# Nikhil-AI-Labs/image-super-resolution-2

Measured on AMD Instinct MI355X. Metric: output MPix/s at x4 SR (256->1024), higher is better.
Workload: dtype bf16 (bf16 MFMA operands, fp32 accumulate, fp32 activations in HBM); 1 GPU; FreqFusion x4 full 3-expert forward (HAT-L + DAT + NAFNet-SR + fusion stack), one 256x256 LR tile -> 1024x1024 per step per GPU (BASELINE configs[1]); seeded synthetic weights (172.3 M params), 1/f-noise tiles; tile=256, parallelism=tile-sharded x1, weights RCCL-broadcast once (0.0 ms), no per-tile collectives, launch=hipGraph replay, tiles_in_flight=2

## Files before the change

image-super-resolution-2_amd/build.py:

```python
from __future__ import annotations

import os
import subprocess
import sys
from concurrent.futures import ThreadPoolExecutor

HERE = os.path.dirname(os.path.abspath(__file__))
CSRC = os.path.join(HERE, "csrc")
LIB = os.path.join(HERE, "libff_hip.so")
SOURCES = ["ff_runtime.hip", "conv_gemm.hip", "conv_gemm_bf16.hip", "gemm_rows_bf16.hip", "conv3x3_halo.hip", "sgfn_tail.hip", "ocab_attn.hip", "conv3x3_small.hip", "attention.hip", "attention_bf16.hip", "win_attn_fused.hip", "chan_qkv.hip", "token_mlp.hip", "token_linear.hip", "naf_fused.hip", "naf_tail.hip", "norm_pool.hip", "dwconv.hip", "elementwise.hip",
           "resample.hip", "freq.hip", "fusion_ops.hip", "metrics.hip", "train_ops.hip", "sr_losses.hip", "augment.hip", "ff_executor.hip"]
HIPCC = os.environ.get("HIPCC", "/opt/rocm/bin/hipcc")
FLAGS = ["--offload-arch=gfx950", "-O3", "-fPIC", "-std=c++17", "-Wall", "-Wno-unused-function", "-I" + os.path.join(HERE, "build")]


def _stale() -> bool:
    if not os.path.exists(LIB):
        return True
    t = os.path.getmtime(LIB)
    deps = [os.path.join(CSRC, f) for f in os.listdir(CSRC)] + [os.path.join(HERE, "..", "include", "ff_kernels.h")]
    return any(os.path.getmtime(d) > t for d in deps)


def gen_dispatch(path: str) -> None:
    from .lib import parse_header
    protos = {n: p for n, p in parse_header().items() if p[1] and p[1][-1] == "void*" and p[0] == "int"
              and n not in ("ff_forward", "ff_create", "ff_upload")}
    names = sorted(protos)
    out = ["// generated by build.py from include/ff_kernels.h -- do not edit", f"#define FF_DISPATCH_COUNT {len(names)}",
           "static const char* const FF_DISPATCH_NAMES[FF_DISPATCH_COUNT] = {" + ", ".join(f'"{n}"' for n in names) + "};"]
    def kinds(n):
        ks = []
        for i, ty in enumerate(protos[n][1]):
            if i == len(protos[n][1]) - 1:
                ks.append("S")
            elif ty.endswith("*"):
                ks.append("P")
            elif ty in ("float", "double"):
                ks.append("F")
            else:
                ks.append("I")
        return "".join(ks)
    out.append("static const char* const FF_DISPATCH_KINDS[FF_DISPATCH_COUNT] = {" + ", ".join(f'"{kinds(n)}"' for n in names) + "};")
    for n in names:
        out.append(f'extern "C" int {n}(' + ", ".join(protos[n][1]) + ");")
    out.append("static int ff_dispatch(int id, const FFVal* v) {\n  switch (id) {")
    for k, n in enumerate(names):
        args = []
        for i, ty in enumerate(protos[n][1]):
            if ty.endswith("*"):
                args.append(f"({ty})v[{i}].p")
            elif ty in ("float", "double"):
                args.append(f"({ty})v[{i}].f")
            else:
                args.append(f"({ty})v[{i}].i")
        out.append(f"    case {k}: return {n}(" + ", ".join(args) + ");")
    out.append('    default: ff_set_error("ff_dispatch: bad entry point id %d", id); return FF_ERR_ARG;\n  }\n}')
    txt = "\n".join(out) + "\n"
    if not os.path.exists(path) or open(path).read() != txt:
        open(path, "w").write(txt)


def build(force: bool = False, verbose: bool = False) -> str:
    objdir = os.path.join(HERE, "build")
    os.makedirs(objdir, exist_ok=True)
    gen_dispatch(os.path.join(objdir, "ff_dispatch_gen.h"))
    if not force and not _stale():
        return LIB

    def cc(src):
        obj = os.path.join(objdir, src.replace(".hip", ".o"))
        cmd = [HIPCC, *FLAGS, "-c", os.path.join(CSRC, src), "-o", obj]
        r = subprocess.run(cmd, capture_output=True, text=True)
        if r.returncode != 0:
            raise RuntimeError(f"hipcc failed for {src}:\n{r.stderr}")
        if verbose and r.stderr:
            print(r.stderr, file=sys.stderr)
        return obj

    with ThreadPoolExecutor(max_workers=min(4, os.cpu_count() or 1)) as ex:
        objs = list(ex.map(cc, SOURCES))
    r = subprocess.run([HIPCC, "--offload-arch=gfx950", "-shared", "-fPIC", "-o", LIB, *objs], capture_output=True, text=True)
    if r.returncode != 0:
        raise RuntimeError(f"link failed:\n{r.stderr}")
    return LIB


if __name__ == "__main__":
    print(build(force="--force" in sys.argv, verbose=True))
```

image-super-resolution-2_amd/csrc/token_mlp.hip:

```cpp
#include "ff_common.h"

#define TM_KP 192
#define TM_NP 192
#define TM_KS 12
#define W1SLOTS 25
#define W2SLOTS 5
#define W1ROWB (W1SLOTS * 16)
#define W2ROWB (W2SLOTS * 16)
#define W1PL (32 * W1SLOTS)
#define W2PL (TM_NP * W2SLOTS)
#define W1PIECES (2 * W1PL / 64)
#define W2PIECES (2 * W2PL / 64)
#define TILE_ELEMS 6144
#define XLROWB 400

struct TokenMlpParams {
  const float* x; float* out;
  const float* gamma; const float* beta;
  const __bf16* w;
  const float* b1;
  const float* b2;
  long long M;
  int ldx, ldo, K, N, HT;
  float eps;
};

template <bool VEC4, int NTERMS>
__global__ __launch_bounds__(512) void token_mlp_kernel(TokenMlpParams p) {
  extern __shared__ __attribute__((aligned(16))) unsigned char smem[];
  constexpr int W1B = W1PL * 16, W2B = W2PL * 16;
  unsigned char* W1s = smem;
  unsigned char* W2s = smem + 2 * W1B;
  unsigned char* XLs = smem + 2 * W1B + 2 * W2B;
  float* B1s = reinterpret_cast<float*>(XLs + 8 * 32 * XLROWB);
  const int tid = threadIdx.x, lane = tid & 63, wid = tid >> 6;
  const int l31 = lane & 31, hh = lane >> 5;
  const long long tok = (long long)blockIdx.x * 256 + wid * 32 + l31;
  const bool tvalid = tok < p.M;

  int off1[4], off2[4];
#pragma unroll
  for (int i = 0; i < 4; ++i) {
    int s = (wid + 8 * i) * 64 + lane;
    if (s >= 2 * W1PL) s = 2 * W1PL - 1;
    int plane = s / W1PL, t = s - plane * W1PL, row = t / W1SLOTS, q = t - row * W1SLOTS;
    if (q > 23) q = 23;
    off1[i] = plane * TILE_ELEMS + row * 192 + q * 8;
    s = (wid + 8 * i) * 64 + lane;
    if (s >= 2 * W2PL) s = 2 * W2PL - 1;
    plane = s / W2PL; t = s - plane * W2PL; row = t / W2SLOTS; q = t - row * W2SLOTS;
    if (q > 3) q = 3;
    off2[i] = (2 + plane) * TILE_ELEMS + row * 32 + q * 8;
  }
  auto dma_w1 = [&](int ht) {
    const __bf16* rec = p.w + (long long)ht * (4 * TILE_ELEMS);
#pragma unroll
    for (int i = 0; i < 4; ++i)
      if (wid + 8 * i < W1PIECES)
        __builtin_amdgcn_global_load_lds((const __attribute__((address_space(1))) void*)(rec + off1[i]),
                                         (__attribute__((address_space(3))) void*)(W1s + (wid + 8 * i) * 1024), 16, 0, 0);
  };
  auto dma_w2 = [&](int ht) {
    const __bf16* rec = p.w + (long long)ht * (4 * TILE_ELEMS);
#pragma unroll
    for (int i = 0; i < 4; ++i)
      if (wid + 8 * i < W2PIECES)
        __builtin_amdgcn_global_load_lds((const __attribute__((address_space(1))) void*)(rec + off2[i]),
                                         (__attribute__((address_space(3))) void*)(W2s + (wid + 8 * i) * 1024), 16, 0, 0);
  };
  dma_w1(0);
  dma_w2(0);
  for (int i = tid; i < p.HT * 32; i += 512) B1s[i] = p.b1[i];

  bf16x8 xh[TM_KS];
  unsigned char* xl_row = XLs + (size_t)(wid * 32 + l31) * XLROWB + 16 * hh;
  {
    float v[TM_KS][8];
    ff_wave_rows_to_frags<3>(p.x, p.ldx, (long long)blockIdx.x * 256 + wid * 32, p.M, p.K,
                          reinterpret_cast<float*>(XLs + (size_t)wid * 32 * XLROWB), lane, v);
    float mean, rstd;
    ff_frag_ln_stats<TM_KS>(v, p.K, hh, p.eps, mean, rstd);
#pragma unroll
    for (int st = 0; st < TM_KS; ++st) {
      float f[8];
      ff_frag_ln_step(v[st], p.gamma, p.beta, 16 * st + 8 * hh, p.K, mean, rstd, f);
      bf16x8 lo;
#pragma unroll
      for (int j = 0; j < 8; ++j) {
        __bf16 h, l;
        ff_bf16_split(f[j], h, l);
        xh[st][j] = h;
        lo[j] = l;
      }
      *reinterpret_cast<bf16x8*>(xl_row + 32 * st) = lo;
    }
  }

// ... 385 lines not shown
        __builtin_amdgcn_sched_barrier(0);
        hacc = __builtin_amdgcn_mfma_f32_32x32x16_bf16(ah, xl, hacc, 0, 0, 0);
        hacc = __builtin_amdgcn_mfma_f32_32x32x16_bf16(al, xh[st], hacc, 0, 0, 0);
        hacc = __builtin_amdgcn_mfma_f32_32x32x16_bf16(ah, xh[st], hacc, 0, 0, 0);
        __builtin_amdgcn_sched_barrier(0);
      }
    }
    if (ht < 3) FF_STAMP(64, 8 + 4 * ht);
    asm volatile("s_waitcnt vmcnt(0)" ::: "memory");
    __syncthreads();
    if (ht < 3) FF_STAMP(64, 9 + 4 * ht);
    if (ht + 1 < p.HT) dma_w1(ht + 1);
    bf16x8 gh[2], gl[2];
#pragma unroll
    for (int s = 0; s < 2; ++s)
#pragma unroll
      for (int j = 0; j < 8; ++j) {
        const float g = ff_gelu_fast(hacc[8 * s + j]);
        const __bf16 h = (__bf16)g;
        gh[s][j] = h;
        gl[s][j] = (__bf16)(g - (float)h);
      }
    {
      const unsigned char* ap = W2s + l31 * W2ROWB + 16 * hh;
      bf16x8 fa[2], fl[2];
#pragma unroll
      for (int u = 0; u < 2; ++u) {
        fa[u] = *reinterpret_cast<const bf16x8*>(ap + (u >> 1) * 32 * W2ROWB + 32 * (u & 1));
        fl[u] = *reinterpret_cast<const bf16x8*>(ap + (u >> 1) * 32 * W2ROWB + 32 * (u & 1) + W2B);
      }
#pragma unroll
      for (int u = 0; u < 12; ++u) {
        const int n = u >> 1, s2 = u & 1;
        const bf16x8 ah = fa[u & 1], al = fl[u & 1];
        if (u + 2 < 12) {
          fa[u & 1] = *reinterpret_cast<const bf16x8*>(ap + ((u + 2) >> 1) * 32 * W2ROWB + 32 * ((u + 2) & 1));
          fl[u & 1] = *reinterpret_cast<const bf16x8*>(ap + ((u + 2) >> 1) * 32 * W2ROWB + 32 * ((u + 2) & 1) + W2B);
        }
        __builtin_amdgcn_sched_barrier(0);
        oacc[n] = __builtin_amdgcn_mfma_f32_32x32x16_bf16(ah, gl[s2], oacc[n], 0, 0, 0);
        oacc[n] = __builtin_amdgcn_mfma_f32_32x32x16_bf16(al, gh[s2], oacc[n], 0, 0, 0);
        oacc[n] = __builtin_amdgcn_mfma_f32_32x32x16_bf16(ah, gh[s2], oacc[n], 0, 0, 0);
        __builtin_amdgcn_sched_barrier(0);
      }
    }
    if (ht < 3) FF_STAMP(64, 10 + 4 * ht);
    asm volatile("s_waitcnt vmcnt(0)" ::: "memory");
    __syncthreads();
    if (ht < 3) FF_STAMP(64, 11 + 4 * ht);
    if (ht + 1 < p.HT) dma_w2(ht + 1);
  }
  FF_STAMP(64, 40);

  {
    float* tr = reinterpret_cast<float*>(smem) + wid * (32 * 36);
    const int tq = lane >> 3, q4 = 4 * (lane & 7);
#pragma unroll
    for (int n = 0; n < 6; ++n) {
      const int c4 = n * 32 + q4;
      const bool cok = c4 < p.N;
      const f32x4 b4 = *reinterpret_cast<const f32x4*>(p.b2 + (cok ? c4 : 0));
#pragma unroll
      for (int g = 0; g < 4; ++g) {
        f32x4 v4;
#pragma unroll
        for (int e = 0; e < 4; ++e) v4[e] = oacc[n][4 * g + e];
        *reinterpret_cast<f32x4*>(tr + l31 * 36 + 8 * g + 4 * hh) = v4;
      }
      f32x4 ov[4];
#pragma unroll
      for (int i = 0; i < 4; ++i) ov[i] = *reinterpret_cast<const f32x4*>(tr + (tq + 8 * i) * 36 + q4) + b4;
      if (cok) {
        float* op = p.out + (tok0 + tq) * p.ldo + c4;
#pragma unroll
        for (int i = 0; i < 4; ++i)
          if (tok0 + tq + 8 * i < p.M) *reinterpret_cast<f32x4*>(op + (long long)(8 * i) * p.ldo) = ov[i];
      }
    }
  }
  FF_STAMP(64, 41);
  FF_STAMP_DRAINED(64, 42);
}

#define PM_W1SLOT (13 * 1024)
#define PM_W2SLOT (15 * 1024)
#define PM_OFF_W2 (2 * PM_W1SLOT)
#define PM_PROJB (6 * PM_W1SLOT)
#define PM_PATCHB (32 * FF_XS_ROW * 4)
#define PM_OFF_PATCH PM_PROJB
#define PM_OFF_VEC (PM_OFF_PATCH + 8 * PM_PATCHB)

__global__ __launch_bounds__(512) void token_projmlp_bf16_kernel(TokenProjMlpParams p) {
  extern __shared__ __attribute__((aligned(16))) unsigned char smem[];
  float* Gs = reinterpret_cast<float*>(smem + PM_OFF_VEC);
  float* Bts = Gs + TM_KP;
  float* B1s = Bts + TM_KP;
  const int tid = threadIdx.x, lane = tid & 63, wid = tid >> 6;
  const int l31 = lane & 31, hh = lane >> 5;
  const long long tok0 = ((long long)blockIdx.y * p.wpi + blockIdx.x) * 256 + wid * 32;
  float* patch = reinterpret_cast<float*>(smem + PM_OFF_PATCH + wid * PM_PATCHB);
  FF_STAMP(64, 0);

#pragma unroll
  for (int i = 0; i < 10; ++i) {
    const int pc = wid + 8 * i;
    if (pc < 78) {
      const int tile = pc / 13, pw = pc - 13 * tile;
      int s = pw * 64 + lane;
      if (s > W1PL - 1) s = W1PL - 1;
      const int row = s / W1SLOTS;
      int q = s - row * W1SLOTS;
      if (q > 23) q = 23;
      __builtin_amdgcn_global_load_lds((const __attribute__((address_space(1))) void*)(p.wp + (long long)tile * (2 * TILE_ELEMS) + row * 192 + q * 8),
                                       (__attribute__((address_space(3))) void*)(smem + pc * 1024), 16, 0, 0);
    }
  }
  int off1[2], off2[2];
#pragma unroll
  for (int i = 0; i < 2; ++i) {
    int s = (wid + 8 * i) * 64 + lane;
    if (s > W1PL - 1) s = W1PL - 1;
    int row = s / W1SLOTS, q = s - row * W1SLOTS;
    if (q > 23) q = 23;
    off1[i] = row * 192 + q * 8;
    s = (wid + 8 * i) * 64 + lane;
    if (s > W2PL - 1) s = W2PL - 1;
    row = s / W2SLOTS; q = s - row * W2SLOTS;
    if (q > 3) q = 3;
    off2[i] = 2 * TILE_ELEMS + row * 32 + q * 8;
  }
  auto dma_mlp = [&](int ht, int slot) {
    const __bf16* rec = p.w + (long long)ht * (4 * TILE_ELEMS);
#pragma unroll
    for (int i = 0; i < 2; ++i) {
      if (wid + 8 * i < 13)
        __builtin_amdgcn_global_load_lds((const __attribute__((address_space(1))) void*)(rec + off1[i]),
                                         (__attribute__((address_space(3))) void*)(smem + slot * PM_W1SLOT + (wid + 8 * i) * 1024), 16, 0, 0);
      if (wid + 8 * i < 15)
        __builtin_amdgcn_global_load_lds((const __attribute__((address_space(1))) void*)(rec + off2[i]),
                                         (__attribute__((address_space(3))) void*)(smem + PM_OFF_W2 + slot * PM_W2SLOT + (wid + 8 * i) * 1024), 16, 0, 0);
    }
  };
  for (int i = tid; i < p.HT * 32; i += 512) B1s[i] = p.b1[i];
  if (tid < TM_KP) { Gs[tid] = tid < p.K ? p.gamma[tid] : 0.f; Bts[tid] = tid < p.K ? p.beta[tid] : 0.f; }

  bf16x8 xh[TM_KS];
  if (p.io_bf16 & 1) {
    const long long tk = tok0 + l31 < p.M ? tok0 + l31 : 0;
    const __bf16* arow = reinterpret_cast<const __bf16*>(p.att) + tk * p.lda + 8 * hh;
#pragma unroll
    for (int st = 0; st < TM_KS; ++st) {
      xh[st] = *reinterpret_cast<const bf16x8*>(arow + 16 * st);
      if (16 * st + 8 * hh + 7 >= p.K) {
#pragma unroll
        for (int j = 0; j < 8; ++j)
          if (16 * st + 8 * hh + j >= p.K) xh[st][j] = (__bf16)0.f;
      }
    }
  } else {
    float v[TM_KS][8];
    ff_wave_rows_to_frags<3>(p.att, p.lda, tok0, p.M, p.K, patch, lane, v);
#pragma unroll
    for (int st = 0; st < TM_KS; ++st)
#pragma unroll
      for (int j = 0; j < 8; ++j) xh[st][j] = (__bf16)v[st][j];
  }
  FF_STAMP(64, 1);

  const int tq = lane >> 3, q4 = 4 * (lane & 7);
  f32x4 rx[4], rc[4];
  int xo[4], co[4];
#pragma unroll
  for (int i = 0; i < 4; ++i) {
// ... 23 lines not shown
#pragma unroll
    for (int r = 0; r < 16; ++r) oacc[n][r] = bpn[(r & 3) + 8 * (r >> 2)];
    const unsigned char* ap = smem + n * PM_W1SLOT + l31 * W1ROWB + 16 * hh;
    bf16x8 fa[2];
#pragma unroll
    for (int u = 0; u < 2; ++u) fa[u] = *reinterpret_cast<const bf16x8*>(ap + 32 * u);
#pragma unroll
    for (int st = 0; st < TM_KS; ++st) {
      const bf16x8 ah = fa[st & 1];
      if (st + 2 < TM_KS) fa[st & 1] = *reinterpret_cast<const bf16x8*>(ap + 32 * (st + 2));
      __builtin_amdgcn_sched_barrier(0);
      oacc[n] = __builtin_amdgcn_mfma_f32_32x32x16_bf16(ah, xh[st], oacc[n], 0, 0, 0);
      __builtin_amdgcn_sched_barrier(0);
    }
  }
  FF_STAMP(64, 2);
  asm volatile("s_waitcnt lgkmcnt(0)" ::: "memory");
  __builtin_amdgcn_s_barrier();
  FF_STAMP(64, 3);
  dma_mlp(0, 0);
  if (p.HT > 1) dma_mlp(1, 1);
#pragma unroll
  for (int n = 0; n < 6; ++n) {
    {
      load_res(n);
      const int c4 = n * 32 + q4;
      f32x4 sc = {0.f, 0.f, 0.f, 0.f};
      if (p.c2 && c4 < p.N) sc = *reinterpret_cast<const f32x4*>(p.rs2 + (long long)blockIdx.y * p.rs2_ld + c4);
#pragma unroll
      for (int i = 0; i < 4; ++i) {
        f32x4 r0 = rx[i];
        if (p.c2) r0 += rc[i] * sc;
        *reinterpret_cast<f32x4*>(patch + (tq + 8 * i) * 36 + q4) = r0;
      }
#pragma unroll
      for (int g = 0; g < 4; ++g) {
        const f32x4 u = *reinterpret_cast<const f32x4*>(patch + l31 * 36 + 8 * g + 4 * hh);
#pragma unroll
        for (int e = 0; e < 4; ++e) oacc[n][4 * g + e] += u[e];
      }
    }
  }
  FF_STAMP(64, 4);

  {
    float s = 0.f;
#pragma unroll
    for (int n = 0; n < 6; ++n)
#pragma unroll
      for (int r = 0; r < 16; ++r) s += (n * 32 + (r & 3) + 8 * (r >> 2) + 4 * hh < p.K) ? oacc[n][r] : 0.f;
    s += __shfl_xor(s, 32);
    const float mean = s / (float)p.K;
    float qv = 0.f;
#pragma unroll
    for (int n = 0; n < 6; ++n)
#pragma unroll
      for (int r = 0; r < 16; ++r) {
        const float d = (n * 32 + (r & 3) + 8 * (r >> 2) + 4 * hh < p.K) ? oacc[n][r] - mean : 0.f;
        qv += d * d;
      }
    qv += __shfl_xor(qv, 32);
    const float rstd = 1.0f / sqrtf(qv / (float)p.K + p.eps);
#pragma unroll
    for (int n = 0; n < 6; ++n)
#pragma unroll
      for (int s2 = 0; s2 < 2; ++s2) {
#pragma unroll
        for (int g2 = 0; g2 < 2; ++g2) {
          const int c0 = n * 32 + 8 * (2 * s2 + g2) + 4 * hh;
          const f32x4 g4 = *reinterpret_cast<const f32x4*>(Gs + c0);
          const f32x4 b4 = *reinterpret_cast<const f32x4*>(Bts + c0);
#pragma unroll
          for (int e = 0; e < 4; ++e)
            xh[2 * n + s2][4 * g2 + e] = (__bf16)((oacc[n][8 * s2 + 4 * g2 + e] - mean) * rstd * g4[e] + b4[e]);
        }
        asm volatile("" : "+v"(xh[2 * n + s2]) :: "memory");
      }
  }
  FF_STAMP(64, 5);
  asm volatile("s_waitcnt vmcnt(0) lgkmcnt(0)" ::: "memory");
  __builtin_amdgcn_s_barrier();
  FF_STAMP(64, 6);

  for (int ht = 0; ht < p.HT; ++ht) {
    const int slot = ht & 1;
    f32x16 hacc;
#pragma unroll
    for (int r = 0; r < 16; ++r) hacc[r] = B1s[ht * 32 + (r & 3) + 8 * (r >> 2) + 4 * hh];
    {
      const unsigned char* ap = smem + slot * PM_W1SLOT + l31 * W1ROWB + 16 * hh;
      bf16x8 fa[2];
#pragma unroll
      for (int u = 0; u < 2; ++u) fa[u] = *reinterpret_cast<const bf16x8*>(ap + 32 * u);
#pragma unroll
      for (int st = 0; st < TM_KS; ++st) {
        const bf16x8 ah = fa[st & 1];
        if (st + 2 < TM_KS) fa[st & 1] = *reinterpret_cast<const bf16x8*>(ap + 32 * (st + 2));
        __builtin_amdgcn_sched_barrier(0);
        hacc = __builtin_amdgcn_mfma_f32_32x32x16_bf16(ah, xh[st], hacc, 0, 0, 0);
        __builtin_amdgcn_sched_barrier(0);
      }
    }
    if (ht < 3) FF_STAMP(64, 8 + 4 * ht);
    bf16x8 gh[2];
#pragma unroll
    for (int s = 0; s < 2; ++s)
#pragma unroll
      for (int j = 0; j < 8; j += 2) {
        const f32x2 g = ff_gelu_sig2((f32x2){hacc[8 * s + j], hacc[8 * s + j + 1]});
        gh[s][j] = (__bf16)g[0];
        gh[s][j + 1] = (__bf16)g[1];
      }
    if (ht < 3) FF_STAMP(64, 9 + 4 * ht);
    {
      const unsigned char* ap = smem + PM_OFF_W2 + slot * PM_W2SLOT + l31 * W2ROWB + 16 * hh;
      bf16x8 fa[2];
#pragma unroll
      for (int u = 0; u < 2; ++u) fa[u] = *reinterpret_cast<const bf16x8*>(ap + (u >> 1) * 32 * W2ROWB + 32 * (u & 1));
#pragma unroll
      for (int u = 0; u < 12; ++u) {
        const int n = u >> 1, s2 = u & 1;
        const bf16x8 ah = fa[u & 1];
        if (u + 2 < 12) fa[u & 1] = *reinterpret_cast<const bf16x8*>(ap + ((u + 2) >> 1) * 32 * W2ROWB + 32 * ((u + 2) & 1));
        __builtin_amdgcn_sched_barrier(0);
        oacc[n] = __builtin_amdgcn_mfma_f32_32x32x16_bf16(ah, gh[s2], oacc[n], 0, 0, 0);
        __builtin_amdgcn_sched_barrier(0);
      }
    }
    if (ht < 3) FF_STAMP(64, 10 + 4 * ht);
    asm volatile("s_waitcnt vmcnt(0) lgkmcnt(0)" ::: "memory");
    __builtin_amdgcn_s_barrier();
    if (ht < 3) FF_STAMP(64, 11 + 4 * ht);
    if (ht + 2 < p.HT) dma_mlp(ht + 2, slot);
  }
  FF_STAMP(64, 40);

  {
#pragma unroll
    for (int n = 0; n < 6; ++n) {
      const int c4 = n * 32 + q4;
      const bool cok = c4 < p.N;
      const f32x4 b4 = *reinterpret_cast<const f32x4*>(p.b2 + (cok ? c4 : 0));
#pragma unroll
      for (int g = 0; g < 4; ++g) {
        f32x4 v4;
#pragma unroll
        for (int e = 0; e < 4; ++e) v4[e] = oacc[n][4 * g + e];
        *reinterpret_cast<f32x4*>(patch + l31 * 36 + 8 * g + 4 * hh) = v4;
      }
      f32x4 ov[4];
#pragma unroll
      for (int i = 0; i < 4; ++i) ov[i] = *reinterpret_cast<const f32x4*>(patch + (tq + 8 * i) * 36 + q4) + b4;
      if (cok) {
        float* op = p.out + (tok0 + tq) * p.ldo + c4;
#pragma unroll
        for (int i = 0; i < 4; ++i)
          if (tok0 + tq + 8 * i < p.M) *reinterpret_cast<f32x4*>(op + (long long)(8 * i) * p.ldo) = ov[i];
      }
    }
  }
  FF_STAMP(64, 41);
  FF_STAMP_DRAINED(64, 42);
}

static int token_projmlp_launch(const float* att, int lda, const float* x, int ldx, const float* c2, int ldc, const float* c2_scale,
                                int scale_ld, int images, float* out, int ldo, long long M, int K, int hidden_tiles, const void* proj_tiles,
                                const float* proj_bias_padded, const float* gamma, const float* beta, float eps,
                                const void* mlp_tiles, const float* b1_padded, const float* b2, int nterms, int io_bf16, void* stream) {
  FF_CHECK_ARG(nterms == 1 || nterms == 3, "ff_token_projmlp: nterms must be 1 or 3");
  FF_CHECK_ARG(io_bf16 == 0 || (nterms == 1 && io_bf16 > 0 && io_bf16 < 4), "ff_token_projmlp: bf16 att / c2 rows exist for nterms == 1 only");
  FF_CHECK_ARG(!(io_bf16 & 1) || (lda % 8 == 0 && lda >= ((K + 15) / 16) * 16), "ff_token_projmlp: bf16 att rows must be 16-byte aligned and padded to a multiple of 16 channels");
  FF_CHECK_ARG(att && x && out && proj_tiles && proj_bias_padded && gamma && beta && mlp_tiles && b1_padded && b2, "ff_token_projmlp: null pointer");
  FF_CHECK_ARG(M > 0 && K > 0 && K <= TM_KP && K % 4 == 0 && hidden_tiles > 0, "ff_token_projmlp: needs K <= 192 (K %% 4 == 0)");
  FF_CHECK_ARG(lda >= K && lda % 4 == 0 && ldx >= K && ldx % 4 == 0 && ldo >= K && ldo % 4 == 0, "ff_token_projmlp: rows must be 16-byte aligned");
  FF_CHECK_ARG((((uintptr_t)att) & 15) == 0 && (((uintptr_t)x) & 15) == 0 && (((uintptr_t)out) & 15) == 0, "ff_token_projmlp: 16-byte aligned tensors");
  FF_CHECK_ARG((c2 == nullptr) == (c2_scale == nullptr), "ff_token_projmlp: c2 / c2_scale come together");
  FF_CHECK_ARG(!c2 || (ldc >= K && ldc % 4 == 0 && (((uintptr_t)c2) & 15) == 0 && (((uintptr_t)c2_scale) & 15) == 0), "ff_token_projmlp: c2 rows must be 16-byte aligned");
  FF_CHECK_ARG((((uintptr_t)proj_tiles) & 15) == 0 && (((uintptr_t)mlp_tiles) & 15) == 0 && (((uintptr_t)gamma) & 15) == 0 &&
               (((uintptr_t)beta) & 15) == 0 && (((uintptr_t)b2) & 15) == 0, "ff_token_projmlp: weights / gamma / beta / b2 must be 16-byte aligned");
  TokenProjMlpParams p;
  p.att = att; p.x = x; p.c2 = c2; p.rs2 = c2_scale; p.out = out; p.gamma = gamma; p.beta = beta;
  p.wp = (const __bf16*)proj_tiles; p.bp = proj_bias_padded; p.w = (const __bf16*)mlp_tiles; p.b1 = b1_padded; p.b2 = b2;
  p.M = M; p.lda = lda; p.ldx = ldx; p.ldc = ldc; p.ldo = ldo; p.K = K; p.N = K; p.HT = hidden_tiles; p.eps = eps; p.io_bf16 = io_bf16;
  p.wpi = (int)(((M + 255) / 256) / images); p.rs2_ld = images > 1 ? scale_ld : 0;
  FF_STAMP_ARM(p);
  const size_t lds = (size_t)(2 * W1PL + 2 * W2PL) * 16 + (size_t)8 * 32 * XLROWB + (size_t)hidden_tiles * 32 * 4;
  FF_CHECK_ARG(lds <= 160 * 1024, "ff_token_projmlp: hidden too large for the LDS image");
  const long long nblk = (M + 255) / 256;
  const dim3 grid((unsigned)(nblk / images), (unsigned)images);
  FF_CHECK_ARG(nblk < (1LL << 31), "ff_token_projmlp: grid too large");
  FF_CHECK_ARG(M * (long long)(ldx > ldc ? ldx : ldc) < (1LL << 31), "ff_token_projmlp: too many tokens for 32-bit row offsets");
  static bool attr_set = false;
  if (!attr_set) {
    hipError_t e = hipFuncSetAttribute(reinterpret_cast<const void*>(&token_projmlp_kernel), hipFuncAttributeMaxDynamicSharedMemorySize, 160 * 1024);
    if (e != hipSuccess) { ff_set_error("ff_token_projmlp: cannot raise dynamic LDS: %s", hipGetErrorString(e)); return FF_ERR_LAUNCH; }
    attr_set = true;
  }
  if (nterms == 1) {
    const size_t lds2 = (size_t)PM_OFF_VEC + (size_t)(2 * TM_KP + hidden_tiles * 32) * 4;
    FF_CHECK_ARG(lds2 <= 160 * 1024, "ff_token_projmlp: hidden too large for the LDS image");
    static bool attr2 = false;
    if (!attr2) {
      hipError_t e = hipFuncSetAttribute(reinterpret_cast<const void*>(&token_projmlp_bf16_kernel), hipFuncAttributeMaxDynamicSharedMemorySize, 160 * 1024);
      if (e != hipSuccess) { ff_set_error("ff_token_projmlp: cannot raise dynamic LDS: %s", hipGetErrorString(e)); return FF_ERR_LAUNCH; }
      attr2 = true;
    }
    hipLaunchKernelGGL(token_projmlp_bf16_kernel, grid, dim3(512), lds2, (hipStream_t)stream, p);
  } else hipLaunchKernelGGL(token_projmlp_kernel, grid, dim3(512), lds, (hipStream_t)stream, p);
  FF_LAUNCH_CHECK("ff_token_projmlp");
  return FF_OK;
}

extern "C" int ff_token_projmlp(const float* att, int lda, const float* x, int ldx, const float* c2, int ldc, const float* c2_scale,
                                float* out, int ldo, long long M, int K, int hidden_tiles, const void* proj_tiles,
                                const float* proj_bias_padded, const float* gamma, const float* beta, float eps,
                                const void* mlp_tiles, const float* b1_padded, const float* b2, int nterms, int io_bf16, void* stream) {
  return token_projmlp_launch(att, lda, x, ldx, c2, ldc, c2_scale, 0, 1, out, ldo, M, K, hidden_tiles, proj_tiles, proj_bias_padded, gamma, beta,
// ... 51 lines not shown
```

image-super-resolution-2_amd/csrc/win_attn_fused.hip:

```cpp
#include "ff_common.h"

struct WinFusedParams {
  const float* x; float* out;
  const float* gamma; const float* beta;
  const __bf16* w;
  const float* bias;
  const float* rel;
  float* xn; float* vout;
  int ldx, ldo, ldxn, ldv, o_off, v_off;
  int B, H, W, Hp, Wp, sh, sw, use_mask, nwx, nwy;
  int head0, nheads, d, K, zero_pad, rel_rows, rel_stride;
  int out_bf16, xn_bf16;
  float eps;
  FF_STAMP_MEMBER
};

#define WF_KS 12
#define WF_SLOTS 25
#define WF_ROWB (WF_SLOTS * 16)
#define WF_PL (32 * WF_SLOTS)
#define WF_PLB (WF_PL * 16)
#define WF_BUFB (2 * WF_PLB)
#define WF_TILE_ELEMS (32 * 192)
#define WF_KROWB 80
#define WF_KWAVE (2 * 32 * WF_KROWB)
#define WF_VROWB 528
#define WF_VPLB (32 * WF_VROWB)
#define WF_OFF_K (2 * WF_BUFB)
#define WF_OFF_V (WF_OFF_K + 8 * WF_KWAVE)
#define WF_OFF_REL (WF_OFF_V + 2 * WF_VPLB)
#define WF_REL_MAX 2560
#define WF_REL_PAD 4
#define WF_OFF_BS (WF_OFF_REL + (WF_REL_MAX + WF_REL_PAD) * 4)
#define WF_BS_MAX 576
#define WF_OFF_TOK (WF_OFF_BS + WF_BS_MAX * 4)
#define WF_OFF_REG (WF_OFF_TOK + 1024)
#define WF_OFF_SAME (WF_OFF_REG + 1024)
#define WF_LDS (WF_OFF_SAME + 9 * 8 * 4)
#define WF_XS_ROW 68

template <int WW, int NTERMS>
__global__ __launch_bounds__(512) void win_attn_fused_kernel(WinFusedParams p) {
  constexpr int WH = 256 / WW;
  constexpr int RS = WW == 8 ? 40 : (WW == 16 ? 48 : 64);
  constexpr int CMAX = (WH - 1) * RS + WW - 1;
  extern __shared__ __attribute__((aligned(16))) unsigned char smem[];
  unsigned char* KB = smem + WF_OFF_K;
  unsigned char* VB = smem + WF_OFF_V;
  float* REL = reinterpret_cast<float*>(smem + WF_OFF_REL);
  float* Bs = reinterpret_cast<float*>(smem + WF_OFF_BS);
  int* ktok = reinterpret_cast<int*>(smem + WF_OFF_TOK);
  int* kreg = reinterpret_cast<int*>(smem + WF_OFF_REG);
  unsigned* same = reinterpret_cast<unsigned*>(smem + WF_OFF_SAME);

  const int tid = threadIdx.x, lane = tid & 63, wid = tid >> 6;
  const int l31 = lane & 31, hh = lane >> 5;
  int bid = blockIdx.x;
  const int wx = bid % p.nwx; bid /= p.nwx;
  const int wy = bid % p.nwy;
  const int b = bid / p.nwy;
  FF_STAMP(64, 0);

  int off[4];
#pragma unroll
  for (int i = 0; i < 4; ++i) {
    int s = (wid + 8 * i) * 64 + lane;
    if (s >= 2 * WF_PL) s = 2 * WF_PL - 1;
    const int plane = s / WF_PL, t = s - plane * WF_PL, row = t / WF_SLOTS;
    int q = t - row * WF_SLOTS;
    if (q > 2 * WF_KS - 1) q = 2 * WF_KS - 1;
    off[i] = plane * WF_TILE_ELEMS + row * 192 + q * 8;
  }
  auto dma = [&](int tile, int buf) {
    const __bf16* rec = p.w + (long long)tile * (2 * WF_TILE_ELEMS);
#pragma unroll
    for (int i = 0; i < 4; ++i)
      if (wid + 8 * i < 25)
        __builtin_amdgcn_global_load_lds((const __attribute__((address_space(1))) void*)(rec + off[i]),
                                         (__attribute__((address_space(3))) void*)(smem + buf * WF_BUFB + (wid + 8 * i) * 1024), 16, 0, 0);
  };
  const int tile0 = 3 * p.head0, ntiles = 3 * p.nheads;
  dma(tile0, 0);

  if (tid < 256) {
    const int qy = wy * WH + tid / WW, qx = wx * WW + tid % WW;
    int oy = qy + p.sh, ox = qx + p.sw;
    if (oy >= p.Hp) oy -= p.Hp;
    if (ox >= p.Wp) ox -= p.Wp;
    ktok[tid] = (oy < p.H && ox < p.W) ? (b * p.H + oy) * p.W + ox : -1;
    int rid = 0;
    if (p.use_mask) {
      const int ry = qy < p.Hp - WH ? 0 : (qy < p.Hp - p.sh ? 1 : 2);
      const int rx = qx < p.Wp - WW ? 0 : (qx < p.Wp - p.sw ? 1 : 2);
      rid = 3 * ry + rx;
    }
    kreg[tid] = rid;
  }
  for (int i = tid; i < ntiles * 32; i += 512) Bs[i] = p.bias ? p.bias[tile0 * 32 + i] : 0.f;
  __syncthreads();

  const bool blk_mask = p.use_mask && (wy == p.nwy - 1 || wx == p.nwx - 1);
  if (blk_mask) {
    for (int i = wid; i < 72; i += 8) {
      const int region = i >> 3, t = i & 7;
      const unsigned long long bal = __ballot(l31 == lane && kreg[32 * t + l31] == region);
      if (lane == 0) same[i] = (unsigned)bal;
    }
    __syncthreads();
  }
  const int qi = wid * 32 + l31;
  const int mytok = ktok[qi];
  const bool tvalid = mytok >= 0;
  const int qreg_id = kreg[qi];
  const unsigned vmask = (unsigned)(__ballot(tvalid) & 0xffffffffu);
  const bool kill_pad = p.zero_pad != 0;
  FF_STAMP(64, 1);

  bf16x8 xh[WF_KS], xl[WF_KS];
  {
    float* xs = reinterpret_cast<float*>(smem + WF_OFF_K) + wid * (32 * WF_XS_ROW);
    const int rr = lane >> 4, cq = (lane & 15) * 4;
    float v[WF_KS][8];
// ... 355 lines not shown
```

image-super-resolution-2_amd/csrc/win_attn_fused_v2.inc:

```
#define W2_TILEB (32 * WF_ROWB)
#define W2_HEAD_SLOTS (3 * WF_PL)
#define W2_PIECES ((W2_HEAD_SLOTS + 63) / 64)
#define W2_WB (W2_PIECES * 1024)
#define W2_KROWB 80
#define W2_KWAVE (32 * W2_KROWB)
#define W2_KBUF (8 * W2_KWAVE)
#define W2_VROWB 528
#define W2_VBUF (32 * W2_VROWB)
#define W2_RELB ((WF_REL_MAX + WF_REL_PAD) * 4)
#define W2_OFF_K W2_WB
#define W2_OFF_V (W2_OFF_K + 2 * W2_KBUF)
#define W2_OFF_REL (W2_OFF_V + 2 * W2_VBUF)
#define W2_OFF_BS (W2_OFF_REL + 2 * W2_RELB)
#define W2_OFF_TOK (W2_OFF_BS + WF_BS_MAX * 4)
#define W2_OFF_REG (W2_OFF_TOK + 1024)
#define W2_OFF_SAME (W2_OFF_REG + 1024)
#define W2_LDS (W2_OFF_SAME + 9 * 8 * 4)

template <int WW, bool ONES>
__global__ __launch_bounds__(512) void win_attn_fused_v2_kernel(WinFusedParams p) {
  constexpr int WH = 256 / WW;
  constexpr int RS = WW == 8 ? 40 : (WW == 16 ? 48 : 64);
  constexpr int TPR = WW >= 32 ? 1 : 32 / WW;
  constexpr int WWM = WW >= 32 ? 32 : WW;
  extern __shared__ __attribute__((aligned(16))) unsigned char smem[];
  float* Bs = reinterpret_cast<float*>(smem + W2_OFF_BS);
  int* ktok = reinterpret_cast<int*>(smem + W2_OFF_TOK);
  int* kreg = reinterpret_cast<int*>(smem + W2_OFF_REG);
  unsigned* same = reinterpret_cast<unsigned*>(smem + W2_OFF_SAME);

  const int tid = threadIdx.x, lane = tid & 63, wid = tid >> 6;
  const int l31 = lane & 31, hh = lane >> 5;
  int bid = blockIdx.x;
  const int wx = bid % p.nwx; bid /= p.nwx;
  const int wy = bid % p.nwy;
  const int b = bid / p.nwy;
  FF_STAMP(64, 0);

  int woff[5];
#pragma unroll
  for (int i = 0; i < 5; ++i) {
    int s = (wid + 8 * i) * 64 + lane;
    if (s >= W2_HEAD_SLOTS) s = W2_HEAD_SLOTS - 1;
    const int tile = s / WF_PL, t = s - tile * WF_PL, row = t / WF_SLOTS;
    int q = t - row * WF_SLOTS;
    if (q > 2 * WF_KS - 1) q = 2 * WF_KS - 1;
    woff[i] = tile * (2 * WF_TILE_ELEMS) + row * 192 + q * 8;
  }
  const int reln = p.rel_rows * p.rel_stride;
  const int relpieces = (reln + 255) >> 8;
  auto dma_head = [&](int head, int buf) {
    const __bf16* rec = p.w + (long long)(3 * head) * (2 * WF_TILE_ELEMS);
#pragma unroll
    for (int i = 0; i < 5; ++i)
      if (wid + 8 * i < W2_PIECES)
        __builtin_amdgcn_global_load_lds((const __attribute__((address_space(1))) void*)(rec + woff[i]),
                                         (__attribute__((address_space(3))) void*)(smem + (wid + 8 * i) * 1024), 16, 0, 0);
    const float* src = p.rel + (long long)head * reln;
#pragma unroll
    for (int i = 0; i < 2; ++i)
      if (wid + 8 * i < relpieces) {
        int c = (wid + 8 * i) * 64 + lane;
        if (c > (reln >> 2) - 1) c = (reln >> 2) - 1;
        __builtin_amdgcn_global_load_lds((const __attribute__((address_space(1))) void*)(src + 4 * c),
                                         (__attribute__((address_space(3))) void*)(smem + W2_OFF_REL + buf * W2_RELB + WF_REL_PAD * 4 + (wid + 8 * i) * 1024), 16, 0, 0);
      }
  };
  dma_head(p.head0, 0);

  if (tid < 256) {
    const int qy = wy * WH + tid / WW, qx = wx * WW + tid % WW;
    int oy = qy + p.sh, ox = qx + p.sw;
    if (oy >= p.Hp) oy -= p.Hp;
    if (ox >= p.Wp) ox -= p.Wp;
    ktok[tid] = (oy < p.H && ox < p.W) ? (b * p.H + oy) * p.W + ox : -1;
    int rid = 0;
    if (p.use_mask) {
      const int ry = qy < p.Hp - WH ? 0 : (qy < p.Hp - p.sh ? 1 : 2);
      const int rx = qx < p.Wp - WW ? 0 : (qx < p.Wp - p.sw ? 1 : 2);
      rid = 3 * ry + rx;
    }
    kreg[tid] = rid;
  }
  for (int i = tid; i < 3 * p.nheads * 32; i += 512) Bs[i] = p.bias ? p.bias[3 * p.head0 * 32 + i] : 0.f;
  __syncthreads();
  if (ONES && tid < p.nheads) Bs[(3 * tid + 2) * 32 + 30] = 1.0f;

  const bool blk_mask = p.use_mask && (wy == p.nwy - 1 || wx == p.nwx - 1);
  if (!ONES && blk_mask) {
    for (int i = wid; i < 72; i += 8) {
      const int region = i >> 3, t = i & 7;
      const unsigned long long bal = __ballot(l31 == lane && kreg[32 * t + 31 - l31] == region);
      if (lane == 0) same[i] = (unsigned)bal;
    }
    __syncthreads();
  }
  const int qi = wid * 32 + 31 - l31;
  const int mytok = ktok[qi];
  const bool tvalid = mytok >= 0;
  const int qreg_id = kreg[qi];
  const unsigned vmask = (unsigned)(__ballot(tvalid) & 0xffffffffu);
  const bool kill_pad = p.zero_pad != 0;
  const float msy = (qreg_id / 3 == 2) ? -7.0625f : 7.0625f, msx = (qreg_id % 3 == 2) ? -7.0625f : 7.0625f;
  FF_STAMP(64, 1);

  bf16x8 xh[WF_KS];
  {
    float* xs = reinterpret_cast<float*>(smem + W2_OFF_K) + wid * (32 * WF_XS_ROW);
    const int rr = lane >> 4, cq = (lane & 15) * 4;
    float v[WF_KS][8];
    f32x4 t[3][8];
#pragma unroll
    for (int pass = 0; pass < 3; ++pass)
#pragma unroll
      for (int j = 0; j < 8; ++j) {
        const int r = 4 * j + rr, c = 64 * pass + cq;
        const int tk = ktok[wid * 32 + r];
        const bool ok = tk >= 0 && c < p.K;
        const f32x4 u = *reinterpret_cast<const f32x4*>(p.x + (ok ? (long long)tk * p.ldx + c : 0));
        t[pass][j] = ok ? u : (f32x4){0.f, 0.f, 0.f, 0.f};
      }
    const float* xrow = xs + (31 - l31) * WF_XS_ROW + 8 * hh;
#pragma unroll
    for (int pass = 0; pass < 3; ++pass) {
#pragma unroll
      for (int j = 0; j < 8; ++j) *reinterpret_cast<f32x4*>(xs + (4 * j + rr) * WF_XS_ROW + cq) = t[pass][j];
#pragma unroll
      for (int s4 = 0; s4 < 4; ++s4) {
        const f32x4 a = *reinterpret_cast<const f32x4*>(xrow + 16 * s4);
        const f32x4 c4 = *reinterpret_cast<const f32x4*>(xrow + 16 * s4 + 4);
#pragma unroll
        for (int e = 0; e < 4; ++e) { v[4 * pass + s4][e] = a[e]; v[4 * pass + s4][4 + e] = c4[e]; }
      }
    }
    asm volatile("s_waitcnt vmcnt(0)" ::: "memory");
    float mean = 0.f, rstd = 1.f;
    if (p.gamma) {
      float s = 0.f;
#pragma unroll
      for (int st = 0; st < WF_KS; ++st)
#pragma unroll
        for (int j = 0; j < 8; ++j) s += v[st][j];
      s += __shfl_xor(s, 32);
      mean = s / (float)p.K;
      float qv = 0.f;
#pragma unroll
      for (int st = 0; st < WF_KS; ++st)
#pragma unroll
        for (int j = 0; j < 8; ++j) {
          const float dd = (16 * st + 8 * hh + j < p.K) ? v[st][j] - mean : 0.f;
          qv += dd * dd;
        }
      qv += __shfl_xor(qv, 32);
      rstd = 1.0f / sqrtf(qv / (float)p.K + p.eps);
    }
#pragma unroll
    for (int st = 0; st < WF_KS; ++st) {
      const int k0 = 16 * st + 8 * hh;
      f32x4 g0 = {1.f, 1.f, 1.f, 1.f}, g1 = g0, b0 = {0.f, 0.f, 0.f, 0.f}, b1 = b0;
      if (p.gamma) {
        const int ka = k0 < p.K ? k0 : 0, kb = k0 + 4 < p.K ? k0 + 4 : 0;
        g0 = *reinterpret_cast<const f32x4*>(p.gamma + ka); b0 = *reinterpret_cast<const f32x4*>(p.beta + ka);
        g1 = *reinterpret_cast<const f32x4*>(p.gamma + kb); b1 = *reinterpret_cast<const f32x4*>(p.beta + kb);
      }
#pragma unroll
      for (int j = 0; j < 8; ++j) {
        const float gg = j < 4 ? g0[j & 3] : g1[j & 3], bb = j < 4 ? b0[j & 3] : b1[j & 3];
        const float f = (k0 + j < p.K) ? (p.gamma ? (v[st][j] - mean) * rstd * gg + bb : v[st][j]) : 0.f;
        xh[st][j] = (__bf16)f;
        v[st][j] = f;
      }
      if (p.xn && tvalid && p.xn_bf16) {
        if (k0 < p.K) *reinterpret_cast<bf16x8*>(reinterpret_cast<__bf16*>(p.xn) + (long long)mytok * p.ldxn + k0) = xh[st];
      } else if (p.xn && tvalid) {
        float* xr = p.xn + (long long)mytok * p.ldxn + k0;
        if (k0 < p.K) *reinterpret_cast<f32x4*>(xr) = (f32x4){v[st][0], v[st][1], v[st][2], v[st][3]};
        if (k0 + 4 < p.K) *reinterpret_cast<f32x4*>(xr + 4) = (f32x4){v[st][4], v[st][5], v[st][6], v[st][7]};
      }
    }
  }
  FF_STAMP(64, 2);

  const int rel_lane = ((qi / WW) + WH - 1) * RS + (qi % WW) + WW - 1 - (TPR - 1) * RS - (WWM - 1) + 4 * hh;
  const float LOG2E = 1.4426950408889634f;

  auto gemm_tile = [&](int j, bool swap, f32x16& acc) {
    const unsigned char* ap = smem + j * W2_TILEB + l31 * WF_ROWB + 16 * hh;
    bf16x8 fa[2];
#pragma unroll
    for (int u = 0; u < 2; ++u) fa[u] = *reinterpret_cast<const bf16x8*>(ap + 32 * u);
#pragma unroll
    for (int st = 0; st < WF_KS; ++st) {
      const bf16x8 ah = fa[st & 1];
      if (st + 2 < WF_KS) fa[st & 1] = *reinterpret_cast<const bf16x8*>(ap + 32 * (st + 2));
      __builtin_amdgcn_sched_barrier(0);
      if (!swap) acc = __builtin_amdgcn_mfma_f32_32x32x16_bf16(ah, xh[st], acc, 0, 0, 0);
      else acc = __builtin_amdgcn_mfma_f32_32x32x16_bf16(xh[st], ah, acc, 0, 0, 0);
      __builtin_amdgcn_sched_barrier(0);
    }
  };

  for (int hi = 0; hi < p.nheads; ++hi) {
    const int g = p.head0 + hi, buf = hi & 1;
    unsigned char* KB = smem + W2_OFF_K + buf * W2_KBUF;
    unsigned char* VB = smem + W2_OFF_V + buf * W2_VBUF;
    asm volatile("s_waitcnt lgkmcnt(0)" ::: "memory");
    __builtin_amdgcn_s_barrier();
    FF_STAMP(64, 3 + 8 * hi);
    bf16x8 qh[2];
    {
      f32x16 acc;
      const int nb = (3 * hi) * 32 + 4 * hh;
#pragma unroll
      for (int r = 0; r < 16; ++r) acc[r] = Bs[nb + (r & 3) + 8 * (r >> 2)];
      gemm_tile(0, false, acc);
      if (ONES && blk_mask && hh) { acc[14] = msy; acc[15] = msx; }
#pragma unroll
      for (int s = 0; s < 2; ++s)
#pragma unroll
        for (int j = 0; j < 8; ++j) qh[s][j] = (__bf16)acc[8 * s + j];
    }
    FF_STAMP(64, 4 + 8 * hi);
    {
      f32x16 acc;
      const int nb = (3 * hi + 1) * 32 + 4 * hh;
#pragma unroll
      for (int r = 0; r < 16; ++r) acc[r] = Bs[nb + (r & 3) + 8 * (r >> 2)];
      gemm_tile(1, false, acc);
      const bool zero = kill_pad && !tvalid;
      if (zero) {
#pragma unroll
        for (int r = 0; r < 16; ++r) acc[r] = 0.f;
      }
      if (ONES && blk_mask && hh) { acc[14] = msy; acc[15] = msx; }
      unsigned char* kmine = KB + wid * W2_KWAVE + l31 * W2_KROWB + 16 * hh;
#pragma unroll
      for (int s = 0; s < 2; ++s) {
        bf16x8 h8;
#pragma unroll
        for (int j = 0; j < 8; ++j) h8[j] = (__bf16)acc[8 * s + j];
        *reinterpret_cast<bf16x8*>(kmine + 32 * s) = h8;
      }
    }
    FF_STAMP(64, 5 + 8 * hi);
    {
      f32x16 acc;
      const float bv = Bs[(3 * hi + 2) * 32 + l31];
#pragma unroll
      for (int r = 0; r < 16; ++r) acc[r] = bv;
      gemm_tile(2, true, acc);
      if (kill_pad && !(ONES && l31 == 30)) {
#pragma unroll
        for (int r = 0; r < 16; ++r)
          if (!((vmask >> ((r & 3) + 8 * (r >> 2) + 4 * hh)) & 1u)) acc[r] = 0.f;
      }
      unsigned char* vp = VB + l31 * W2_VROWB + 64 * wid + 16 * hh;
#pragma unroll
      for (int s = 0; s < 2; ++s) {
        bf16x8 h8;
#pragma unroll
        for (int j = 0; j < 8; ++j) h8[j] = (__bf16)acc[8 * s + j];
        *reinterpret_cast<bf16x8*>(vp + 32 * s) = h8;
      }
      if (p.vout && l31 < p.d) {
#pragma unroll
        for (int r = 0; r < 16; ++r) {
          const int tk = ktok[wid * 32 + 31 - ((r & 3) + 8 * (r >> 2) + 4 * hh)];
          if (tk >= 0) p.vout[(long long)tk * p.ldv + p.v_off + g * p.d + l31] = acc[r];
        }
      }
    }
    FF_STAMP(64, 6 + 8 * hi);
    asm volatile("s_waitcnt lgkmcnt(0)" ::: "memory");
    __builtin_amdgcn_s_barrier();
    FF_STAMP(64, 7 + 8 * hi);
    if (hi + 1 < p.nheads) dma_head(g + 1, buf ^ 1);

    f32x16 o;
#pragma unroll
    for (int r = 0; r < 16; ++r) o[r] = 0.f;
    float m_run = -INFINITY, l_run = 0.f;
    unsigned rel_addr = (unsigned)(size_t)(__attribute__((address_space(3))) const void*)(smem + W2_OFF_REL + buf * W2_RELB + WF_REL_PAD * 4) + 4u * (unsigned)rel_lane;
    const unsigned char* kp = KB + l31 * W2_KROWB + 16 * hh;
    const unsigned char* vq = VB + l31 * W2_VROWB + 16 * hh;
    const unsigned* samep = same + 8 * qreg_id;
#pragma unroll 2
    for (int t = 0; t < 8; ++t, rel_addr -= 4u * TPR * RS, kp += W2_KWAVE, vq += 64) {
      unsigned ra = rel_addr;
      asm volatile("" : "+v"(ra));
      const ff_lds_cf relp = (ff_lds_cf)(size_t)ra;
      f32x16 st;
#pragma unroll
      for (int r = 0; r < 16; ++r) {
        const int c = (r & 3) + 8 * (r >> 2);
        st[r] = relp[(c / WW) * RS + (c % WW)];
      }
      bf16x8 vh2[2];
#pragma unroll
      for (int s = 0; s < 2; ++s) vh2[s] = *reinterpret_cast<const bf16x8*>(vq + 32 * s);
#pragma unroll
      for (int s = 0; s < 2; ++s) {
        const bf16x8 ah = *reinterpret_cast<const bf16x8*>(kp + 32 * s);
        st = __builtin_amdgcn_mfma_f32_32x32x16_bf16(ah, qh[s], st, 0, 0, 0);
      }
      if (!ONES && blk_mask) {
        const unsigned m = samep[t] >> (4 * hh);
#pragma unroll
        for (int r = 0; r < 16; ++r)
          st[r] += ((m >> ((r & 3) + 8 * (r >> 2))) & 1u) ? 0.f : -100.0f;
      }
      float mx = st[0];
#pragma unroll
      for (int r = 1; r < 16; ++r) mx = fmaxf(mx, st[r]);
      {
        float lo, hi;
        ff_halves(mx, lo, hi);
        mx = fmaxf(lo, hi);
      }
      if (__builtin_amdgcn_ballot_w64(mx > m_run) != 0) {
        const float m_new = fmaxf(m_run, mx);
        const float corr = __builtin_amdgcn_exp2f((m_run - m_new) * LOG2E);
#pragma unroll
        for (int r = 0; r < 16; ++r) o[r] *= corr;
        if (!ONES) l_run *= corr;
        m_run = m_new;
      }
      const float mneg = -m_run * LOG2E;
      float ls = 0.f;
#pragma unroll
      for (int s = 0; s < 2; ++s) {
        bf16x8 ph;
#pragma unroll
        for (int j = 0; j < 8; ++j) {
          const float e = __builtin_amdgcn_exp2f(__builtin_fmaf(st[8 * s + j], LOG2E, mneg));
          if (!ONES) ls += e;
          ph[j] = (__bf16)e;
        }
        o = __builtin_amdgcn_mfma_f32_32x32x16_bf16(vh2[s], ph, o, 0, 0, 0);
      }
      if (!ONES) l_run += ls;
    }
    float den;
    if (ONES) {
      float lo;
      ff_halves(o[14], lo, den);
    } else {
      den = l_run + __shfl_xor(l_run, 32);
    }
    const float inv = 1.0f / den;
    FF_STAMP(64, 8 + 8 * hi);
    asm volatile("s_waitcnt vmcnt(0)" ::: "memory");
    FF_STAMP(64, 9 + 8 * hi);

    if (tvalid && p.out_bf16) {
      typedef __bf16 bf16x2 __attribute__((ext_vector_type(2)));
      __bf16* orow = reinterpret_cast<__bf16*>(p.out) + (long long)mytok * p.ldo + p.o_off + g * p.d + 4 * hh;
#pragma unroll
      for (int i = 0; i < 4; ++i) {
        const int c = 8 * i + 4 * hh;
        if (c < p.d) *reinterpret_cast<bf16x2*>(orow + 8 * i) = (bf16x2){(__bf16)(o[4 * i] * inv), (__bf16)(o[4 * i + 1] * inv)};
        if (c + 2 < p.d) *reinterpret_cast<bf16x2*>(orow + 8 * i + 2) = (bf16x2){(__bf16)(o[4 * i + 2] * inv), (__bf16)(o[4 * i + 3] * inv)};
      }
    } else if (tvalid) {
      float* orow = p.out + (long long)mytok * p.ldo + p.o_off + g * p.d + 4 * hh;
#pragma unroll
      for (int i = 0; i < 4; ++i) {
        const int c = 8 * i + 4 * hh;
        if (c < p.d) *reinterpret_cast<float2*>(orow + 8 * i) = (float2){o[4 * i] * inv, o[4 * i + 1] * inv};
        if (c + 2 < p.d) *reinterpret_cast<float2*>(orow + 8 * i + 2) = (float2){o[4 * i + 2] * inv, o[4 * i + 3] * inv};
      }
    }
    FF_STAMP(64, 10 + 8 * hi);
  }
  FF_STAMP(64, 60);
  FF_STAMP_DRAINED(64, 61);
}
```

image-super-resolution-2_amd/experts.py:

```python
from __future__ import annotations

from typing import Dict, List, Optional

import torch

from . import ops
from .prep import (pack_conv, pack_dw, bn_scale_shift, fold_bn_after_conv, pack_token_linear, pack_naf_ffn, pack_naf_tail,
                   pack_win_attn, pack_win_rel, pack_token_projmlp, pack_chan_qkv, pack_token_linear_gated, pack_rel_overlap, pack_ocab_qkv)

T = torch.Tensor
SD = Dict[str, T]
RGB_MEAN = (0.4488, 0.4371, 0.4040)


def _ceil_to(n: int, m: int) -> int:
    return (n + m - 1) // m * m


class _Weights:

    def __init__(self, sd: SD, dev, prefix: str):
        self.sd, self.dev, self.p = sd, dev, prefix

    def __call__(self, name: str) -> T:
# ... 91 lines not shown
        self.pe_norm = (w("patch_embed.norm.weight"), w("patch_embed.norm.bias"))
        self.blocks: List[List[dict]] = []
        self.ocab: List[dict] = []
        self.gconv = []
        for g in range(groups):
            blks = []
            for b in range(depth):
                q = f"layers.{g}.residual_group.blocks.{b}."
                tbl = w(q + "attn.relative_position_bias_table")
                bias = tbl[rpi_sa].reshape(n, n, heads).permute(2, 1, 0).contiguous()
                blks.append(dict(rel=tbl.t().contiguous(),
                    n1=(w(q + "norm1.weight"), w(q + "norm1.bias")), qkv=lin(q + "attn.qkv"), proj=lin(q + "attn.proj"),
                    bias=bias, cab0=(w.conv(q + "conv_block.cab.0"), w(q + "conv_block.cab.0.bias")),
                    cab2=(w.conv(q + "conv_block.cab.2"), w(q + "conv_block.cab.2.bias")),
                    ca1=(w(q + "conv_block.cab.3.attention.1.weight").reshape(-1, 180).contiguous(), w(q + "conv_block.cab.3.attention.1.bias")),
                    ca2=(w(q + "conv_block.cab.3.attention.3.weight").reshape(180, -1).contiguous(), w(q + "conv_block.cab.3.attention.3.bias")),
                    n2=(w(q + "norm2.weight"), w(q + "norm2.bias")), fc1=lin(q + "mlp.fc1"), fc2=lin(q + "mlp.fc2"),
                    shift=0 if b % 2 == 0 else ws // 2))
            self.blocks.append(blks)
            q = f"layers.{g}.residual_group.overlap_attn."
            tbl = w(q + "relative_position_bias_table")
            self.ocab.append(dict(
                n1=(w(q + "norm1.weight"), w(q + "norm1.bias")), qkv=lin(q + "qkv"), proj=lin(q + "proj"),
                bias=tbl[rpi_oca].reshape(n, nk, heads).permute(2, 1, 0).contiguous(), rel=pack_rel_overlap(tbl, ws, self.ows),
                n2=(w(q + "norm2.weight"), w(q + "norm2.bias")), fc1=lin(q + "mlp.fc1"), fc2=lin(q + "mlp.fc2")))
            self.gconv.append((w.conv(f"layers.{g}.conv"), w(f"layers.{g}.conv.bias")))

    def _mlp(self, x: T, blk: dict) -> T:
        xn = ops.layernorm(x, *blk["n2"])
        h = ops.linear(xn, *blk["fc1"], act="gelu")
        return ops.linear(h, *blk["fc2"], res=x)

    def hab(self, x: T, blk: dict) -> T:
        _, H, W, C = x.shape
        d = C // self.heads
        fused = ops.fused_modes()
        b16 = ops.gemm_mode() == "bf16" and H * W >= 1024 and C % 4 == 0
        att = ops.empty_rows_bf16(tuple(x.shape), x.device) if b16 else ops.empty_like_rows(x)
        s = blk["shift"]
        if fused:
            relp = _packed(blk, "relp", lambda: pack_win_rel(blk["rel"], self.ws, self.ws))
            _, xn = ops.win_attn_fused(x, att, _wf(blk, self.heads, d), relp, gamma=blk["n1"][0], beta=blk["n1"][1], H=H, W=W,
                                       Hp=H, Wp=W, win=(self.ws, self.ws), shift=(s, s), use_mask=s > 0, want_xn="bf16" if b16 else True)
        else:
            xn = ops.layernorm(x, *blk["n1"])
            qkv = ops.linear(xn, *blk["qkv"])
            ops.window_attn(qkv, att, blk["bias"], q_off=0, k_off=C, v_off=2 * C, o_off=0, H=H, W=W, Hp=H, Wp=W, win=(self.ws, self.ws),
                            kwin=(self.ws, self.ws), shift=(s, s), use_mask=s > 0, heads=self.heads, d=d, scale=d ** -0.5)
        c1 = ops.conv2d(xn, *blk["cab0"], ksize=(3, 3), pad=(1, 1), act="gelu", out_bf16=b16, per_image=True)
        c2, c2mean = ops.conv2d(c1, *blk["cab2"], ksize=(3, 3), pad=(1, 1), want_pool="partials", out_bf16=b16)
        gate = ops.vec_mlp(c2mean, *blk["ca1"], "relu", *blk["ca2"], "sigmoid", post=self.conv_scale)
        if fused:
            return ops.token_projmlp(att, x, _pm(blk), blk["n2"][0], blk["n2"][1], c2=c2, c2_scale=gate if x.shape[0] > 1 else gate.reshape(-1))
        t = ops.mix2(x, c2, cb=gate)
        x = ops.linear(att, *blk["proj"], res=t)
        return self._mlp(x, blk)

    def ocab_block(self, x: T, blk: dict) -> T:
        _, H, W, C = x.shape
        d = C // self.heads
        fused = ops.fused_modes()
        rows16 = ops.gemm_mode() == "bf16" and (self.ws, self.ows, d) == (16, 24, 30) and H % 16 == 0 and W % 16 == 0
        if rows16:
            pk = _packed(blk, "qkv_r16", lambda: pack_ocab_qkv(*blk["qkv"], self.heads, d))
            qkv = ops.token_linear_rows16(x, pk, gamma=blk["n1"][0], beta=blk["n1"][1])
        elif fused:
            qkv = ops.token_linear(x, _tl(blk, "qkv"), gamma=blk["n1"][0], beta=blk["n1"][1])
        else:
            qkv = ops.linear(ops.layernorm(x, *blk["n1"]), *blk["qkv"])
        if rows16:
            att = ops.empty_rows_bf16(tuple(x.shape), x.device)
            hp = self.heads * 32
            ops.ocab_attn_rows16(qkv, att, blk["rel"], q_off=0, k_off=hp, v_off=2 * hp, H=H, W=W, heads=self.heads, d=d, ws=self.ws,
                                 ows=self.ows)
        else:
            att = ops.empty_like_rows(x)
            ops.window_attn(qkv, att, blk["bias"], q_off=0, k_off=C, v_off=2 * C, o_off=0, H=H, W=W, Hp=H, Wp=W, win=(self.ws, self.ws),
                            kwin=(self.ows, self.ows), shift=(0, 0), use_mask=False, heads=self.heads, d=d, scale=d ** -0.5)
        if fused:
            return ops.token_projmlp(att, x, _pm(blk), blk["n2"][0], blk["n2"][1])
        x = ops.linear(att, *blk["proj"], res=x)
        return self._mlp(x, blk)

    def group(self, x: T, g: int) -> T:
        y = x
        for blk in self.blocks[g]:
            y = self.hab(y, blk)
        y = self.ocab_block(y, self.ocab[g])
        return ops.conv2d(y, *self.gconv[g], ksize=(3, 3), pad=(1, 1), res=x, per_image=True)

    def forward(self, lr: T, taps: Optional[dict] = None, feats: Optional[dict] = None, out: Optional[T] = None) -> T:
        B, _, h, w = lr.shape
        Hp, Wp = _ceil_to(h, self.ws), _ceil_to(w, self.ws)
        if B > 1:
            if taps is not None:
                raise ops._lib.FFError("HatHIP.forward: taps are recorded for B == 1 only")
            nb = 1
            if ops.fused_modes():
                nb = max(1, min(int(self.max_batch_tokens) // (Hp * Wp), (2 ** 31 - 1) // (16 * Hp * Wp * 64)))
            if nb < B:
                if out is None:
                    out = torch.empty((B, 3, 4 * h, 4 * w), device=lr.device, dtype=torch.float32)
                fall = ops.empty_rows((B, Hp, Wp, self.after[0].shape[0]), lr.device) if feats is not None else None
                for b0 in range(0, B, nb):
                    self._forward_chunk(lr[b0:b0 + nb], None, {} if feats is not None else None, out[b0:b0 + nb],
                                        fall[b0:b0 + nb] if feats is not None else None)
                if feats is not None:
                    feats["hat"] = fall
                return out
        return self._forward_chunk(lr, taps, feats, out, None)

    def _forward_chunk(self, lr: T, taps: Optional[dict], feats: Optional[dict], out: Optional[T], feat_out: Optional[T]) -> T:
        _, _, h, w = lr.shape
        Hp, Wp = _ceil_to(h, self.ws), _ceil_to(w, self.ws)
        feat = self._enter(lr, Hp, Wp)
        x = ops.layernorm(feat, *self.pe_norm)
        for g in range(self.groups):
            if taps is not None and g == 0:
                y = x
                for b, blk in enumerate(self.blocks[0]):
                    y = self.hab(y, blk)
                    taps[f"hat.g0.b{b}"] = y
                y = self.ocab_block(y, self.ocab[0])
                taps["hat.g0.ocab"] = y
                x = ops.conv2d(y, *self.gconv[0], ksize=(3, 3), pad=(1, 1), res=x)
                taps["hat.g0.out"] = x
            else:
                x = self.group(x, g)
        return self._exit(x, feat, h, w, feats, out, feat_out)


def _dat_dpb_bias(sd: SD, p: str, hs: int, wsz: int, heads: int) -> T:
    import torch.nn.functional as F
    ys, xs = torch.meshgrid(torch.arange(1 - hs, hs), torch.arange(1 - wsz, wsz), indexing="ij")
    t = F.linear(torch.stack([ys.reshape(-1), xs.reshape(-1)], dim=1).float(), sd[p + ".pos_proj.weight"].float().cpu(),
                 sd[p + ".pos_proj.bias"].float().cpu())
    for j in ("pos1", "pos2", "pos3"):
        t = F.layer_norm(t, (t.shape[-1],), sd[f"{p}.{j}.0.weight"].float().cpu(), sd[f"{p}.{j}.0.bias"].float().cpu())
        t = F.linear(F.relu(t), sd[f"{p}.{j}.2.weight"].float().cpu(), sd[f"{p}.{j}.2.bias"].float().cpu())
    cy, cx = torch.meshgrid(torch.arange(hs), torch.arange(wsz), indexing="ij")
    cy, cx = cy.reshape(-1), cx.reshape(-1)
    idx = (cy[:, None] - cy[None, :] + hs - 1) * (2 * wsz - 1) + (cx[:, None] - cx[None, :] + wsz - 1)
    n = hs * wsz
    return t[idx.reshape(-1)].reshape(n, n, heads).permute(2, 1, 0).contiguous(), t.t().contiguous()


def dat_should_shift(g: int, b: int) -> bool:
    return (g % 2 == 0 and b > 0 and (b - 2) % 4 == 0) or (g % 2 != 0 and b % 4 == 0)


class DatHIP(_Trunk):

    max_batch_tokens = 262144
    name = "dat"

    def __init__(self, sd: SD, dev, prefix: str = "expert_ensemble.dat.", groups: int = 6, depth: int = 6, split=(8, 32),
                 heads: int = 6):
        w = _Weights(sd, dev, prefix)
        self.dev, self.groups, self.depth, self.split, self.heads = dev, groups, depth, split, heads
        self._load_trunk(w, dev)
        C = 180

        def lin(name):
            return w(name + ".weight"), w(name + ".bias")

        def folded_1x1(conv, bn, cin):
            wt = w(conv + ".weight").reshape(-1, cin)
            sc, sh = bn_scale_shift({k: v.to(dev) for k, v in sd.items() if k.startswith(prefix + bn)}, prefix + bn)
            return fold_bn_after_conv(wt, w(conv + ".bias"), sc, sh)

# ... 273 lines not shown
```

image-super-resolution-2_amd/ops.py:

```python
from __future__ import annotations

from typing import Dict, Optional, Tuple

import torch

from . import lib as _lib

ACT = {None: 0, "none": 0, "gelu": 1, "relu": 2, "lrelu": 3, "sigmoid": 4}
T = torch.Tensor

_PROF = None
_META = [0.0, 0.0]


def _note(flops: float = 0.0, nbytes: float = 0.0):
    _META[0] += flops
    _META[1] += nbytes


def _numel(*ts) -> float:
    return float(sum(t.numel() * (t.element_size() / 4.0) for t in ts if t is not None))


def _instrument(fn):
# ... 592 lines not shown
    xp, ldx, B, h_, w_, K = _nhwc(x, "win_attn_fused.x")
    out_bf16 = out.dtype == torch.bfloat16
    op, ldo, *_ = _nhwc(out, "win_attn_fused.out|bf16ok" if out_bf16 else "win_attn_fused.out")
    xn_bf16 = want_xn == "bf16"
    if (out_bf16 or xn_bf16) and _GEMM_MODE != "bf16":
        raise _lib.FFError("win_attn_fused: bf16 outputs exist for the plain-bf16 contraction mode only")
    if (h_, w_) != (H, W) or tuple(out.shape[:3]) != (B, H, W) or K != pk["K"]:
        raise _lib.FFError("win_attn_fused: x/out dims mismatch")
    nheads = pk["heads"] - head0 if nheads is None else nheads
    if tuple(rel_padded.shape[:2]) != (pk["heads"], 2 * win[0] - 1) or not rel_padded.is_contiguous():
        raise _lib.FFError("win_attn_fused: rel_padded must be [heads][2wh-1][stride]")
    if _GEMM_MODE not in ("bf16x3", "bf16"):
        raise _lib.FFError("win_attn_fused exists for the bf16 contraction modes only")
    xn, xnp, ldxn = None, None, 0
    if want_xn:
        xn = empty_rows_bf16(tuple(x.shape), x.device) if xn_bf16 else empty_like_rows(x)
        xnp, ldxn, _, _ = rows_view(xn, "win_attn_fused.xn|bf16ok" if xn_bf16 else "win_attn_fused.xn")
    vp, ldv = None, 0
    if v_out is not None:
        vp, ldv, vb, vh, vw, _ = _nhwc(v_out, "win_attn_fused.v_out")
        if (vb, vh, vw) != (B, H, W):
            raise _lib.FFError("win_attn_fused: v_out dims mismatch")
    _lib.check(_L().ff_win_attn_fused(xp, ldx, op, ldo, o_off, _ptr(gamma), _ptr(beta), float(eps), pk["w"].data_ptr(),
                                      pk["b"].data_ptr(), rel_padded.data_ptr(), rel_padded.shape[1], rel_padded.shape[2], B, H, W,
                                      Hp, Wp, win[0], win[1], shift[0], shift[1], int(use_mask), head0, nheads, pk["d"], K,
                                      int(zero_pad), xnp, ldxn, vp, ldv, v_off, 1 if _GEMM_MODE == "bf16" else 3, int(out_bf16), int(xn_bf16),
                                      _stream()))
    nwin = B * (Hp // win[0]) * (Wp // win[1])
    _note(2.0 * nwin * 256 * K * 3 * nheads * pk["d"] + 4.0 * nwin * nheads * 256 * 256 * pk["d"],
          4.0 * B * H * W * (K * (1 + (0 if not want_xn else (0.5 if xn_bf16 else 1.0))) + nheads * pk["d"] * ((0.5 if out_bf16 else 1.0) + (1 if v_out is not None else 0))))
    return (out, xn) if want_xn else out


def token_mlp(x: T, gamma: T, beta: T, pk: dict, eps: float = 1e-5) -> T:
    xp, ldx, rows, K = rows_view(x, "token_mlp.x")
    if K != pk["K"] or pk["N"] != K:
        raise _lib.FFError("token_mlp: shape mismatch")
    out = empty_like_rows(x)
    op_, ldo_, _, _ = rows_view(out, "token_mlp.out")
    _lib.check(_L().ff_token_mlp(xp, ldx, op_, ldo_, rows, K, pk["ht"], pk["N"], gamma.data_ptr(), beta.data_ptr(),
                                 float(eps), pk["w"].data_ptr(), pk["b1"].data_ptr(), pk["b2"].data_ptr(), _nterms(), _stream()))
    _note(4.0 * rows * K * pk["ht"] * 32, 8.0 * rows * K)
    return out


def token_projmlp(att: T, x: T, pk: dict, gamma: T, beta: T, *, c2: Optional[T] = None, c2_scale: Optional[T] = None,
                  eps: float = 1e-5) -> T:
    att_bf16 = att.dtype == torch.bfloat16
    c2_bf16 = c2 is not None and c2.dtype == torch.bfloat16
    if (att_bf16 or c2_bf16) and _GEMM_MODE != "bf16":
        raise _lib.FFError("token_projmlp: bf16 att / c2 rows exist for the plain-bf16 contraction mode only")
    ap, lda, rows, K = rows_view(att, "token_projmlp.att|bf16ok" if att_bf16 else "token_projmlp.att")
    xp, ldx, xr, xk = rows_view(x, "token_projmlp.x")
    if xr != rows or xk != K or K != pk["mlp"]["K"]:
        raise _lib.FFError("token_projmlp: shape mismatch")
    cp, ldc = None, 0
    if c2 is not None:
        cp, ldc, cr, ck = rows_view(c2, "token_projmlp.c2|bf16ok" if c2_bf16 else "token_projmlp.c2")
        if cr != rows or ck != K or c2_scale is None:
            raise _lib.FFError("token_projmlp: c2 shape mismatch")
    nimg = 1
    if c2 is not None and c2_scale.numel() != K:
        nimg = int(x.shape[0])
        if c2_scale.dim() != 2 or tuple(c2_scale.shape) != (nimg, K) or not c2_scale.is_contiguous() or rows % nimg:
            raise _lib.FFError(f"token_projmlp: c2_scale must be [{K}] or one row per image [{nimg},{K}], got {tuple(c2_scale.shape)}")
        if (rows // nimg) % 256:
            raise _lib.FFError(f"token_projmlp: a per-image gate needs images of a multiple of 256 rows, got {rows // nimg}")
    out = empty_like_rows(x)
    op_, ldo_, _, _ = rows_view(out, "token_projmlp.out")
    m = pk["mlp"]
    if nimg > 1:
        _lib.check(_L().ff_token_projmlp_images(ap, lda, xp, ldx, cp, ldc, _ptr(c2_scale), K, nimg, rows // nimg, op_, ldo_, rows, K, m["ht"],
                                                pk["proj"]["w"].data_ptr(), pk["proj"]["b"].data_ptr(), gamma.data_ptr(), beta.data_ptr(),
                                                float(eps), m["w"].data_ptr(), m["b1"].data_ptr(), m["b2"].data_ptr(), _nterms(),
                                                (1 if att_bf16 else 0) | (2 if c2_bf16 else 0), _stream()))
    else:
        _lib.check(_L().ff_token_projmlp(ap, lda, xp, ldx, cp, ldc, _ptr(c2_scale), op_, ldo_, rows, K, m["ht"], pk["proj"]["w"].data_ptr(),
                                         pk["proj"]["b"].data_ptr(), gamma.data_ptr(), beta.data_ptr(), float(eps), m["w"].data_ptr(),
                                         m["b1"].data_ptr(), m["b2"].data_ptr(), _nterms(), (1 if att_bf16 else 0) | (2 if c2_bf16 else 0), _stream()))
    _note(2.0 * rows * K * K + 4.0 * rows * K * m["ht"] * 32, 4.0 * rows * K * (2 + (0.5 if att_bf16 else 1.0) + (0 if c2 is None else (0.5 if c2_bf16 else 1.0))))
    return out


def token_linear(x: T, pk: dict, *, gamma: Optional[T] = None, beta: Optional[T] = None, eps: float = 1e-5, act=None,
                 res: Optional[T] = None, res2: Optional[T] = None, res2_scale: Optional[T] = None, want_xn: bool = False,
                 stats_range: Optional[Tuple[int, int]] = None, stats_eps: float = 1e-5):
    xp, ldx, rows, K = rows_view(x, "token_linear.x")
    if K != pk["K"]:
        raise _lib.FFError("token_linear: K mismatch")
    N = pk["N"]
    out = empty_rows(tuple(x.shape[:-1]) + (N,), x.device)
    op, ldo, _, _ = rows_view(out, "token_linear.out")
    rp, ldr, r2p, ldr2 = None, 0, None, 0
    if res is not None:
        rp, ldr, rr, rc = rows_view(res, "token_linear.res")
        if rr != rows or rc != N:
            raise _lib.FFError("token_linear: res shape mismatch")
    if res2 is not None:
        r2p, ldr2, rr, rc = rows_view(res2, "token_linear.res2")
        if rr != rows or rc != N or res2_scale is None or res2_scale.numel() != N:
            raise _lib.FFError("token_linear: res2 shape mismatch")
    xn, xnp, ldxn = None, None, 0
    if want_xn:
        if gamma is None:
            raise _lib.FFError("token_linear: want_xn needs LayerNorm parameters")
        xn = empty_like_rows(x)
        xnp, ldxn, _, _ = rows_view(xn, "token_linear.xn")
    stats, sp, slo, shi = None, None, 0, 0
    if stats_range is not None:
        slo, shi = stats_range
        stats = torch.empty((rows, 2), device=x.device, dtype=torch.float32)
        sp = stats.data_ptr()
    _lib.check(_L().ff_token_linear(xp, ldx, op, ldo, rows, K, pk["kpad"], N, pk["nt"], _ptr(gamma), _ptr(beta), float(eps),
                                    pk["w"].data_ptr(), _ptr(pk["b"]), ACT[act], rp, ldr, r2p, ldr2, _ptr(res2_scale), xnp, ldxn,
                                    sp, slo, shi, float(stats_eps), _nterms(), _stream()))
    _note(2.0 * rows * N * K, 4.0 * (rows * K * (2 if want_xn else 1) + rows * N * (1 + (res is not None) + (res2 is not None))))
    if stats is not None:
        return out, stats
    return (out, xn) if want_xn else out


def token_linear_rows16(x: T, pk: dict, *, gamma: Optional[T] = None, beta: Optional[T] = None, eps: float = 1e-5,
                        out: Optional[T] = None) -> T:
    if _GEMM_MODE != "bf16":
        raise _lib.FFError("token_linear_rows16 exists for the plain-bf16 contraction mode only")
    xp, ldx, rows, K = rows_view(x, "token_linear_rows16.x")
    if K != pk["K"]:
        raise _lib.FFError("token_linear_rows16: K mismatch")
    N = pk["N"]
    if out is None:
        out = empty_rows_bf16(tuple(x.shape[:-1]) + (N,), x.device)
    op, ldo, orows, oc = rows_view(out, "token_linear_rows16.out|bf16ok")
    if out.dtype != torch.bfloat16 or orows != rows or oc != N:
        raise _lib.FFError("token_linear_rows16: out must be bf16 rows [rows, N]")
    _lib.check(_L().ff_token_linear_rows16(xp, ldx, op, ldo, rows, K, pk["kpad"], N, pk["nt"], _ptr(gamma), _ptr(beta), float(eps),
                                           pk["w"].data_ptr(), _ptr(pk["b"]), pk["scale"].data_ptr(), ACT[None], None, 0, None, 0, None,
                                           None, 0, None, 0, 0, 0.0, 1, _stream()))
    _note(2.0 * rows * N * K, 4.0 * rows * K + 2.0 * rows * N)
    return out


def dwconv3_gate_pool(t: T, w_tap: T, bias: T):
    tp, ldi, B, H, W, C2 = _nhwc(t, "dwconv3_gate_pool.t")
    if B < 1 or C2 % 2 or tuple(w_tap.shape) != (9, C2):
        raise _lib.FFError("dwconv3_gate_pool: expects [B,H,W,2C] with B >= 1, [9, 2C] tap-major weights")
    C = C2 // 2
    out = torch.empty((B, H, W, C), device=t.device, dtype=torch.float32)
    pooled = torch.empty((B, C), device=t.device, dtype=torch.float32)
    if B == 1:
        nwork = int(_L().ff_dwconv3_gate_pool_workspace(C))
        work = torch.empty(nwork, device=t.device, dtype=torch.float32)
        _lib.check(_L().ff_dwconv3_gate_pool(tp, ldi, out.data_ptr(), C, H, W, C, w_tap.data_ptr(), bias.data_ptr(), pooled.data_ptr(),
                                             work.data_ptr(), nwork, _stream()))
    else:
        nwork = int(_L().ff_dwconv3_gate_pool_images_workspace(B, C))
        work = torch.empty(nwork, device=t.device, dtype=torch.float32)
        _lib.check(_L().ff_dwconv3_gate_pool_images(tp, ldi, out.data_ptr(), C, B, H, W, C, w_tap.data_ptr(), bias.data_ptr(),
                                                    pooled.data_ptr(), work.data_ptr(), nwork, _stream()))
    _note(2.0 * B * H * W * C2 * 9, 4.0 * B * H * W * (C2 + C))
    return out, pooled


def naf_front(x: T, pk: dict, ln_g: T, ln_b: T, w_tap: T, dw_bias: T, eps: float = 1e-6):
    xp, ldx, B, H, W, C = _nhwc(x, "naf_front.x")
    if B < 1 or C not in (64, 128) or pk["N"] != 2 * C or pk["K"] != C or pk["kpad"] != C or tuple(w_tap.shape) != (9, 2 * C):
        raise _lib.FFError("naf_front: expects [B,H,W,C] with B >= 1, C in (64, 128), conv1 packed as [2C, C], [9, 2C] tap-major weights")
# ... 658 lines not shown
    if p < 1 or p > h or p > w:
        raise _lib.FFError(f"crop_pairs_u8: patch {p} does not fit the {h}x{w} LR image")
    pl = [(int(t_), int(l_)) for t_, l_ in positions]
    if not pl:
        raise _lib.FFError("crop_pairs_u8: no positions given")
    for t_, l_ in pl:
        if not (0 <= t_ <= h - p and 0 <= l_ <= w - p):
            raise _lib.FFError(f"crop_pairs_u8: position ({t_}, {l_}) puts a {p}x{p} patch outside the {h}x{w} LR image")
    K = len(pl)
    pos = torch.tensor(pl, dtype=torch.int32).to(lr_u8.device)
    lr = torch.empty((K, 3, p, p), device=lr_u8.device, dtype=torch.float32)
    hr = torch.empty((K, 3, 4 * p, 4 * p), device=lr_u8.device, dtype=torch.float32)
    _lib.check(_L().ff_crop_pairs_u8(lr_u8.data_ptr(), hr_u8.data_ptr(), h, w, pos.data_ptr(), K, p, lr.data_ptr(), hr.data_ptr(), _stream()))
    _note(0.0, 17.0 * K * 3 * p * p * 5.0)
    return lr, hr


AA_TAPS = 16


def _cubic_aa(x: float) -> float:
    a = -0.5
    x = abs(x)
    if x < 1.0:
        return ((a + 2.0) * x - (a + 3.0)) * x * x + 1.0
    if x < 2.0:
        return ((a * x - 5.0 * a) * x + 8.0 * a) * x - 4.0 * a
    return 0.0


def aa_tables(n_in: int, n_out: int):
    import numpy as np
    if n_out < 1 or n_in < n_out:
        raise _lib.FFError(f"aa_tables: expected 1 <= n_out <= n_in, got {n_in} -> {n_out}")
    s = n_in / n_out
    span = np.zeros((n_out, 2), dtype=np.int32)
    wt = np.zeros((n_out, AA_TAPS), dtype=np.float32)
    for i in range(n_out):
        c = s * (i + 0.5)
        lo = max(int(c - 2.0 * s + 0.5), 0)
        hi = min(int(c + 2.0 * s + 0.5), n_in)
        if hi - lo > AA_TAPS:
            raise _lib.FFError(f"aa_tables: {n_in} -> {n_out} needs {hi - lo} taps, the kernel has {AA_TAPS}")
        raw = [np.float32(_cubic_aa((j + lo - c + 0.5) / s)) for j in range(hi - lo)]
        tot = np.float32(0.0)
        for v in raw:
            tot = np.float32(tot + v)
        span[i] = (lo, hi - lo)
        wt[i, :hi - lo] = [np.float32(v / tot) for v in raw]
    return span, wt


_AA_TABLES: Dict[tuple, Tuple[T, T]] = {}


def _aa_tables_dev(n_in: int, n_out: int, device) -> Tuple[T, T]:
    key = (n_in, n_out, str(device))
    ent = _AA_TABLES.get(key)
    if ent is None:
        if len(_AA_TABLES) >= 64:
            _AA_TABLES.clear()
        span, wt = aa_tables(n_in, n_out)
        ent = _AA_TABLES[key] = (torch.from_numpy(span).to(device), torch.from_numpy(wt).to(device))
    return ent


def resize_aa(x: T, size: Tuple[int, int]) -> T:
    _chk(x, "resize_aa.x")
    if x.dim() != 4 or x.shape[1] != 3 or not x.is_contiguous() or x.numel() == 0:
        raise _lib.FFError("resize_aa: expected a non-empty contiguous [B,3,H,W] tensor")
    B, C, Hi, Wi = x.shape
    Ho, Wo = (int(v) for v in size)
    if Ho < 1 or Wo < 1 or Hi != 4 * Ho or Wi != 4 * Wo:
        raise _lib.FFError(f"resize_aa: only the x1/4 ratio is built: {Hi}x{Wi} -> {Ho}x{Wo} is refused")
    span_w, wt_w = _aa_tables_dev(Wi, Wo, x.device)
    span_h, wt_h = _aa_tables_dev(Hi, Ho, x.device)
    out = torch.empty((B, C, Ho, Wo), device=x.device, dtype=torch.float32)
    _lib.check(_L().ff_resize_aa(x.data_ptr(), out.data_ptr(), B * C, Hi, Wi, Ho, Wo, span_w.data_ptr(), wt_w.data_ptr(),
                                 span_h.data_ptr(), wt_h.data_ptr(), _stream()))
    _note(0.0, 4.0 * B * C * (Hi * Wi + Ho * Wo))
    return out


for _n in ("conv2d", "sgfn_tail", "ocab_attn", "ocab_attn_rows16", "token_linear_rows16", "linear", "win_attn_fused", "token_projmlp", "token_linear_gated", "token_mlp", "token_linear", "pixel_mlp", "dwconv3_gate_pool", "naf_front", "naf_ffn", "naf_tail", "window_attn", "layernorm", "pool_mean", "vec_mlp", "dwconv2d", "dwconv3x3_ln", "mix2", "fma3", "affine",
           "nchw_to_nhwc", "nhwc_to_nchw", "resize", "avgpool2", "dct8_bands", "dwt_pass", "fft_bands", "chan_attn_weights", "chan_qkv_attn",
           "band_mha_core", "band_weight", "freq_guidance", "dynamic_gates", "fuse_blend", "tile_accum", "tile_normalize"):
    globals()[_n] = _instrument(globals()[_n])
```

include/ff_kernels.h:

```cpp
#ifndef FF_KERNELS_H
#define FF_KERNELS_H
#ifdef __cplusplus
extern "C" {
#endif

#define FF_ACT_NONE 0
#define FF_ACT_GELU 1
#define FF_ACT_RELU 2
#define FF_ACT_LRELU 3
#define FF_ACT_SIGMOID 4

const char* ff_last_error(void);
int ff_abi_version(void);
int ff_device_cu_count(void);

int ff_conv2d(const float* in, const float* w, const float* bias, const float* mul, const float* res, float* out,
              int B, int H, int W, int Cin, int ldi, int Ho, int Wo, int Cout, int ldo, int ldr, int KH, int KW,
              int sy, int sx, int py, int px, int act, float alpha, int shuffle, int tile_hint, void* stream);

int ff_conv2d_bf16s(const float* in, const void* w_hi, const void* w_lo, int Kp, int Cp, const float* bias, const float* mul,
                    const float* res, float* out, int B, int H, int W, int Cin, int ldi, int Ho, int Wo, int Cout,
                    int ldo, int ldr, int KH, int KW, int sy, int sx, int py, int px, int act, float alpha, int shuffle,
                    int nterms, int tile_hint, const float* kmul, void* stream);
int ff_conv2d_bf16s_tile(long long M, int Cout, int K, int vec4);
int ff_conv2d_bf16s_kmul_images(const float* in, int ldi, const void* w_hi, const void* w_lo, int Kp, int Cp, const float* kmul, int B,
                                int rows_per_image, const float* bias, const float* mul, const float* res, int ldr, float* out, int ldo,
                                long long M, int Cin, int Cout, int nterms, int tile_hint, void* stream);
int ff_split_bf16(const float* w, int N, int K, int Kp, int Cin, int Cp, void* hi, void* lo, void* stream);

int ff_conv2d_bf16s_wimages(const float* in, int ldi, const void* w_hi, const void* w_lo, int Kp, int Cp, int B, int rows_per_image,
                            const float* bias, const float* mul, const float* res, int ldr, float* out, int ldo, long long M, int Cin,
                            int Cout, int nterms, int tile_hint, void* stream);

int ff_gemm_rows_bf16(const void* a, int a_fp32, int lda, const void* w_hi, int Kp, const float* kmul, const float* bias,
                      const float* mul, const float* res, int ldr, void* out, int ldo, long long M, int N, int K, int gate,
                      int tile_hint, void* stream);
int ff_gemm_rows_bf16_tile(long long M, int N);
int ff_gemm_rows_bf16_kmul_images(const float* a, int lda, const void* w_hi, int Kp, const float* kmul, int B, int rows_per_image,
                                  const float* bias, const float* mul, const float* res, int ldr, float* out, int ldo, long long M,
                                  int N, int K, int tile_hint, void* stream);

int ff_conv3x3_small(const float* in, int ldi, const float* w_small, int ct, const float* bias, const float* res, int ldr,
                     float* out, int ldo, int B, int H, int W, int Cin, int Cout, int act, float alpha, void* stream);


int ff_window_attn(const float* qkv, int ldq, int q_off, int k_off, int v_off, float* out, int ldo, int o_off,
                   const float* biasT, int B, int H, int W, int Hp, int Wp, int wh, int ww, int kh, int kw,
                   int shift_h, int shift_w, int use_mask, int heads, int d, float scale, void* stream);

int ff_window_attn_bf16s(const float* qkv, int ldq, int q_off, int k_off, int v_off, float* out, int ldo, int o_off,
                         const float* biasT, int B, int H, int W, int Hp, int Wp, int wh, int ww, int kh, int kw,
                         int shift_h, int shift_w, int use_mask, int heads, int d, float scale, int nterms, const float* rel_table,
                         void* stream);

int ff_token_projmlp(const float* att, int lda, const float* x, int ldx, const float* c2, int ldc, const float* c2_scale,
                     float* out, int ldo, long long M, int K, int hidden_tiles, const void* proj_tiles,
                     const float* proj_bias_padded, const float* gamma, const float* beta, float eps,
                     const void* mlp_tiles, const float* b1_padded, const float* b2, int nterms, int io_bf16, void* stream);
int ff_token_projmlp_images(const float* att, int lda, const float* x, int ldx, const float* c2, int ldc, const float* c2_scale,
                            int scale_ld, int B, long long rows_per_image, float* out, int ldo, long long M, int K,
                            int hidden_tiles, const void* proj_tiles, const float* proj_bias_padded, const float* gamma,
                            const float* beta, float eps, const void* mlp_tiles, const float* b1_padded, const float* b2,
                            int nterms, int io_bf16, void* stream);

int ff_win_attn_fused(const float* x, int ldx, float* out, int ldo, int o_off, const float* gamma, const float* beta,
                      float eps, const void* w_tiles, const float* bias_padded, const float* rel_padded, int rel_rows,
                      int rel_stride, int B, int H, int W, int Hp, int Wp, int wh, int ww, int shift_h, int shift_w,
                      int use_mask, int head0, int nheads, int d, int K, int zero_pad_tokens, float* xn_out, int ldxn,
                      float* v_out, int ldv, int v_off, int nterms, int out_bf16, int xn_bf16, void* stream);

int ff_token_mlp(const float* x, int ldx, float* out, int ldo, long long M, int K, int hidden_tiles, int N,
                 const float* gamma, const float* beta, float eps, const void* w_tiles, const float* b1_padded,
                 const float* b2, int nterms, void* stream);

long long ff_conv3x3_halo_weight_bytes(int Cout, int Cin, int bn, int nterms);
long long ff_conv3x3_halo_pool_rows(int B, int H, int W, int Cout, int bn, int nterms);
int ff_pool_finish(const float* part, int rows, int ld, int C, float inv_count, float* out, void* stream);
int ff_conv3x3_halo(const float* in, int ldi, const void* w_img, int bn, const float* bias, const float* mul,
                    const float* res, int ldr, float* out, int ldo, int B, int H, int W, int Cin, int Cout,
                    int act, float alpha, int shuffle, float* pool_partials, int nterms, int io_bf16, void* stream);
long long ff_conv3x3_halo_images_pool_rows(int B, int H, int W, int Cout, int bn, int nterms);
int ff_conv3x3_halo_images(const float* in, int ldi, const void* w_img, int bn, const float* bias, const float* mul,
                           const float* res, int ldr, float* out, int ldo, int B, int H, int W, int Cin, int Cout,
                           int act, float alpha, int shuffle, float* pool_partials, int nterms, int io_bf16, void* stream);

int ff_token_linear(const float* x, int ldx, float* out, int ldo, long long M, int K, int kpad, int N, int n_tiles,
                    const float* gamma, const float* beta, float eps, const void* w_tiles, const float* bias_padded,
                    int act, const float* res, int ldr, const float* res2, int ldr2, const float* res2_scale,
                    float* xn_out, int ldxn, float* stats_out, int stat_lo,
                    int stat_hi, float stat_eps, int nterms, void* stream);

int ff_token_linear_rows16(const float* x, int ldx, void* out16, int ldo, long long M, int K, int kpad, int N, int n_tiles,
                           const float* gamma, const float* beta, float eps, const void* w_tiles, const float* bias_padded,
                           const float* col_scale, int act, const float* res, int ldr, const float* res2, int ldr2,
                           const float* res2_scale, float* xn_out, int ldxn, float* stats_out, int stat_lo,
                           int stat_hi, float stat_eps, int nterms, void* stream);

int ff_token_linear_gated(const float* x, int ldx, const float* x2, int ldx2, const float* cm, const float* gw1t, const float* gb1,
                          const float* gw2, float gb2, float* out, int ldo, long long M, int K, int N, int n_tiles,
                          const void* w_tiles, const float* bias_padded, const float* res, int ldr, int nterms, void* stream);
int ff_token_linear_gated_images(const float* x, int ldx, const float* x2, int ldx2, const float* cm, int B, long long rows_per_image,
                                 const float* gb1, const float* gw2, float gb2, float* out, int ldo, long long M, int K, int N, int n_tiles,
                                 const void* w_tiles, const float* bias_padded, const float* res, int ldr, int nterms, void* stream);

long long ff_dwconv3_gate_pool_workspace(int C);
int ff_dwconv3_gate_pool(const float* in, int ldi, float* out, int ldo, int H, int W, int C, const float* w_tapmajor,
                         const float* bias, float* pooled, float* work, long long work_floats, void* stream);
long long ff_dwconv3_gate_pool_images_workspace(int B, int C);
int ff_dwconv3_gate_pool_images(const float* in, int ldi, float* out, int ldo, int B, int H, int W, int C, const float* w_tapmajor,
                                const float* bias, float* pooled, float* work, long long work_floats, void* stream);

long long ff_naf_front_workspace(int H, int W, int C);
int ff_naf_front(const float* x, int ldx, int H, int W, int C, const float* ln_gamma, const float* ln_beta, float eps,
                 const void* w1_tiles, const float* b1, const float* dw_tapmajor, const float* dw_bias, float* out, int ldo,
                 float* pooled, float* work, long long work_floats, int nterms, void* stream);
long long ff_naf_front_images_workspace(int B, int H, int W, int C);
int ff_naf_front_images(const float* x, int ldx, int B, int H, int W, int C, const float* ln_gamma, const float* ln_beta, float eps,
                        const void* w1_tiles, const float* b1, const float* dw_tapmajor, const float* dw_bias, float* out, int ldo,
                        float* pooled, float* work, long long work_floats, int nterms, void* stream);
int ff_naf_ffn(const float* y, int ldy, float* out, int ldo, long long M, int C, const float* gamma_ln, const float* beta_ln,
               float eps, const void* w_tiles, const float* b4, const float* b5, const float* out_scale, int nterms, void* stream);

int ff_naf_tail(const float* g, int ldg, const float* x, int ldx, float* out, int ldo, long long M, int C, const float* sca,
                const float* b3, const float* beta, const float* gamma_ln, const float* beta_ln, float eps, const void* w_frags,
                const float* b4, const float* b5, const float* out_scale, void* stream);
int ff_naf_tail_images(const float* g, int ldg, const float* x, int ldx, float* out, int ldo, long long M, int C, const float* sca,
                       int B, int rows_per_image, const float* b3, const float* beta, const float* gamma_ln, const float* beta_ln,
                       float eps, const void* w_frags, const float* b4, const float* b5, const float* out_scale, void* stream);

int ff_layernorm(const float* in, int ldi, float* out, int ldo, long long rows, int C, const float* gamma,
                 const float* beta, float eps, void* stream);
int ff_layernorm_bf16out(const float* in, int ldi, void* out, int ldo, long long rows, int C, const float* gamma,
                         const float* beta, float eps, void* stream);

int ff_pool_mean(const float* in, int ld, int B, long long P, int C, float* out, float* work, long long work_floats,
                 void* stream);
long long ff_pool_mean_workspace(int B, long long P, int C);

int ff_vec_mlp(const float* in, int B, int Cin, const float* W1, const float* b1, int Ch, int act1, const float* W2,
               const float* b2, int Cout, int act2, float post, float* out, void* stream);

int ff_pool_partial_rows(long long P);
int ff_pool_partials(const float* in, int ld, long long P, int C, float* part, long long part_floats, void* stream);
long long ff_pool_partials_images_rows(int B, long long P);
int ff_pool_partials_images(const float* in, int ld, int B, long long P, int C, float* part, long long part_floats, void* stream);

int ff_pool_vec_mlp(const float* part, int rows, int ld, float inv_count, int Cin, const float* W1, const float* b1, int Ch,
                    int act1, const float* W2, const float* b2, int Cout, int act2, float post, float* out, float* pooled_out,
                    void* stream);
int ff_pool_vec_mlp_images(const float* part, int B, int rows, int ld, float inv_count, int Cin, const float* W1, const float* b1,
                           int Ch, int act1, const float* W2, const float* b2, int Cout, int act2, float post, float* out,
                           float* pooled_out, void* stream);
// ... 184 lines not shown
```

Baseline: 26.81 output MPix/s.

## Fuse HAB tail projection/MLP with next block's window attention in one kernel

Adds a hab_link kernel that runs one HAB block's output projection, residual with the gated CAB branch, LayerNorm and MLP, then continues into the next block's LayerNorm and windowed attention inside the same workgroup. Each workgroup owns one 16x16 window, so the tokens stay in LDS and registers between the two stages. The goal is to drop the HBM round trip of x and the extra launch between blocks. The costs are a very large, specialised kernel limited to six heads of dim 30, K=180 and 16x16 windows, with the shifted-window token mapping applied inside the MLP stage and heavy LDS reuse that could lower occupancy.

```diff
diff --git a/image-super-resolution-2_amd/build.py b/image-super-resolution-2_amd/build.py
--- a/image-super-resolution-2_amd/build.py
+++ b/image-super-resolution-2_amd/build.py
@@ -8,7 +8,7 @@
 HERE = os.path.dirname(os.path.abspath(__file__))
 CSRC = os.path.join(HERE, "csrc")
 LIB = os.path.join(HERE, "libff_hip.so")
-SOURCES = ["ff_runtime.hip", "conv_gemm.hip", "conv_gemm_bf16.hip", "gemm_rows_bf16.hip", "conv3x3_halo.hip", "sgfn_tail.hip", "ocab_attn.hip", "conv3x3_small.hip", "attention.hip", "attention_bf16.hip", "win_attn_fused.hip", "chan_qkv.hip", "token_mlp.hip", "token_linear.hip", "naf_fused.hip", "naf_tail.hip", "norm_pool.hip", "dwconv.hip", "elementwise.hip",
+SOURCES = ["ff_runtime.hip", "conv_gemm.hip", "conv_gemm_bf16.hip", "gemm_rows_bf16.hip", "conv3x3_halo.hip", "sgfn_tail.hip", "ocab_attn.hip", "conv3x3_small.hip", "attention.hip", "attention_bf16.hip", "win_attn_fused.hip", "hab_link.hip", "chan_qkv.hip", "token_mlp.hip", "token_linear.hip", "naf_fused.hip", "naf_tail.hip", "norm_pool.hip", "dwconv.hip", "elementwise.hip",
            "resample.hip", "freq.hip", "fusion_ops.hip", "metrics.hip", "train_ops.hip", "sr_losses.hip", "augment.hip", "ff_executor.hip"]
 HIPCC = os.environ.get("HIPCC", "/opt/rocm/bin/hipcc")
 FLAGS = ["--offload-arch=gfx950", "-O3", "-fPIC", "-std=c++17", "-Wall", "-Wno-unused-function", "-I" + os.path.join(HERE, "build")]
diff --git a/image-super-resolution-2_amd/csrc/hab_link.hip b/image-super-resolution-2_amd/csrc/hab_link.hip
--- /dev/null
+++ b/image-super-resolution-2_amd/csrc/hab_link.hip
@@ -0,0 +1,388 @@
+#include "ff_common.h"
+#include "token_mlp_layout.h"
+#include "win_attn_layout.h"
+
+#define HL_OFF_VEC PM_OFF_VEC
+#define HL_K 180
+#define HL_HEADS 6
+
+struct HabLinkParams {
+  const __bf16* a_att; const float* a_x; const __bf16* a_c2; const float* a_rs2; float* a_out;
+  const float* a_gamma; const float* a_beta; const __bf16* a_wp; const float* a_bp; const __bf16* a_w; const float* a_b1; const float* a_b2;
+  int a_lda, a_ldx, a_ldc, a_ldo, a_rs2_ld, HT;
+  float a_eps;
+  float* out; const float* gamma; const float* beta; const __bf16* w; const float* bias; const float* rel; float* xn;
+  int ldo, ldxn, o_off, H, W, sh, sw, use_mask, nwx, nwy, rel_rows, rel_stride;
+  int K;
+  float eps;
+  static constexpr int d = 30, head0 = 0, nheads = HL_HEADS, out_bf16 = 1, xn_bf16 = 1, ldv = 0, v_off = 0;
+  static constexpr float* vout = nullptr;
+  FF_STAMP_MEMBER
+};
+
+#define HL_LDS (HL_OFF_VEC + (2 * TM_KP + 12 * 32) * 4)
+static_assert(HL_LDS <= 160 * 1024, "LDS image too large");
+static_assert(W2_LDS <= PM_OFF_VEC, "the attention's tables must stay below phase A's vectors");
+static_assert(W2_WB <= PM_PROJB && W2_OFF_K + 8 * 32 * WF_XS_ROW * 4 <= W2_OFF_REL, "hand-over patches must clear the weight image and the bias tables");
+
+__global__ __launch_bounds__(512) void hab_link_kernel(HabLinkParams p) {
+  constexpr int WW = 16, WH = 16, RS = 48, TPR = 2, WWM = 16;
+  constexpr bool ONES = true;
+  extern __shared__ __attribute__((aligned(16))) unsigned char smem[];
+  float* Gs = reinterpret_cast<float*>(smem + HL_OFF_VEC);
+  float* Bts = Gs + TM_KP;
+  float* B1s = Bts + TM_KP;
+  float* Bs = reinterpret_cast<float*>(smem + W2_OFF_BS);
+  unsigned* same = reinterpret_cast<unsigned*>(smem + W2_OFF_SAME);
+  const int* ktok = nullptr;
+  const int tid = threadIdx.x, lane = tid & 63, wid = tid >> 6;
+  const int l31 = lane & 31, hh = lane >> 5;
+  int bid = blockIdx.x;
+  const int wx = bid % p.nwx; bid /= p.nwx;
+  const int wy = bid % p.nwy;
+  const int b = bid / p.nwy;
+  float* patch = reinterpret_cast<float*>(smem + PM_OFF_PATCH + wid * PM_PATCHB);
+  auto tok_of = [&](int pos) {
+    int oy = wy * WH + (pos >> 4) + p.sh, ox = wx * WW + (pos & 15) + p.sw;
+    if (oy >= p.H) oy -= p.H;
+    if (ox >= p.W) ox -= p.W;
+    return (b * p.H + oy) * p.W + ox;
+  };
+  FF_STAMP(128, 0);
+
+#pragma unroll
+  for (int i = 0; i < 10; ++i) {
+    const int pc = wid + 8 * i;
+    if (pc < 78) {
+      const int tile = pc / 13, pw = pc - 13 * tile;
+      int s = pw * 64 + lane;
+      if (s > W1PL - 1) s = W1PL - 1;
+      const int row = s / W1SLOTS;
+      int q = s - row * W1SLOTS;
+      if (q > 23) q = 23;
+      __builtin_amdgcn_global_load_lds((const __attribute__((address_space(1))) void*)(p.a_wp + (long long)tile * (2 * TILE_ELEMS) + row * 192 + q * 8),
+                                       (__attribute__((address_space(3))) void*)(smem + pc * 1024), 16, 0, 0);
+    }
+  }
+  int off1[2], off2[2];
+#pragma unroll
+  for (int i = 0; i < 2; ++i) {
+    int s = (wid + 8 * i) * 64 + lane;
+    if (s > W1PL - 1) s = W1PL - 1;
+    int row = s / W1SLOTS, q = s - row * W1SLOTS;
+    if (q > 23) q = 23;
+    off1[i] = row * 192 + q * 8;
+    s = (wid + 8 * i) * 64 + lane;
+    if (s > W2PL - 1) s = W2PL - 1;
+    row = s / W2SLOTS; q = s - row * W2SLOTS;
+    if (q > 3) q = 3;
+    off2[i] = 2 * TILE_ELEMS + row * 32 + q * 8;
+  }
+  auto dma_mlp = [&](int ht, int slot) {
+    const __bf16* rec = p.a_w + (long long)ht * (4 * TILE_ELEMS);
+#pragma unroll
+    for (int i = 0; i < 2; ++i) {
+      if (wid + 8 * i < 13)
+        __builtin_amdgcn_global_load_lds((const __attribute__((address_space(1))) void*)(rec + off1[i]),
+                                         (__attribute__((address_space(3))) void*)(smem + slot * PM_W1SLOT + (wid + 8 * i) * 1024), 16, 0, 0);
+      if (wid + 8 * i < 15)
+        __builtin_amdgcn_global_load_lds((const __attribute__((address_space(1))) void*)(rec + off2[i]),
+                                         (__attribute__((address_space(3))) void*)(smem + PM_OFF_W2 + slot * PM_W2SLOT + (wid + 8 * i) * 1024), 16, 0, 0);
+    }
+  };
+  for (int i = tid; i < p.HT * 32; i += 512) B1s[i] = p.a_b1[i];
+  if (tid < TM_KP) { Gs[tid] = tid < p.K ? p.a_gamma[tid] : 0.f; Bts[tid] = tid < p.K ? p.a_beta[tid] : 0.f; }
+
+  bf16x8 xh[TM_KS];
+  {
+    const __bf16* arow = p.a_att + tok_of(wid * 32 + l31) * p.a_lda + 8 * hh;
+#pragma unroll
+    for (int st = 0; st < TM_KS; ++st) {
+      xh[st] = *reinterpret_cast<const bf16x8*>(arow + 16 * st);
+      if (16 * st + 8 * hh + 7 >= p.K) {
+#pragma unroll
+        for (int j = 0; j < 8; ++j)
+          if (16 * st + 8 * hh + j >= p.K) xh[st][j] = (__bf16)0.f;
+      }
+    }
+  }
+  FF_STAMP(128, 1);
+
+  const int tq = lane >> 3, q4 = 4 * (lane & 7);
+  f32x4 rx[4], rc[4];
+  int xo[4], co[4];
+#pragma unroll
+  for (int i = 0; i < 4; ++i) {
+    const int t = tok_of(wid * 32 + tq + 8 * i);
+    xo[i] = t * p.a_ldx + q4;
+    co[i] = t * p.a_ldc + q4;
+  }
+  auto load_res = [&](int n) {
+    const int cn = (n * 32 + q4 < p.K) ? n * 32 : -q4;
+#pragma unroll
+    for (int i = 0; i < 4; ++i) {
+      rx[i] = *reinterpret_cast<const f32x4*>(p.a_x + (xo[i] + cn));
+      const bf16x4 h4 = *reinterpret_cast<const bf16x4*>(p.a_c2 + (co[i] + cn));
+      rc[i] = (f32x4){(float)h4[0], (float)h4[1], (float)h4[2], (float)h4[3]};
+    }
+  };
+  asm volatile("s_waitcnt vmcnt(0) lgkmcnt(0)" ::: "memory");
+  __builtin_amdgcn_s_barrier();
+
+  f32x16 oacc[6];
+#pragma unroll
+  for (int n = 0; n < 6; ++n) {
+    const float* bpn = p.a_bp + n * 32 + 4 * hh;
+#pragma unroll
+    for (int r = 0; r < 16; ++r) oacc[n][r] = bpn[(r & 3) + 8 * (r >> 2)];
+    const unsigned char* ap = smem + n * PM_W1SLOT + l31 * W1ROWB + 16 * hh;
+    bf16x8 fa[2];
+#pragma unroll
+    for (int u = 0; u < 2; ++u) fa[u] = *reinterpret_cast<const bf16x8*>(ap + 32 * u);
+#pragma unroll
+    for (int st = 0; st < TM_KS; ++st) {
+      const bf16x8 ah = fa[st & 1];
+      if (st + 2 < TM_KS) fa[st & 1] = *reinterpret_cast<const bf16x8*>(ap + 32 * (st + 2));
+      __builtin_amdgcn_sched_barrier(0);
+      oacc[n] = __builtin_amdgcn_mfma_f32_32x32x16_bf16(ah, xh[st], oacc[n], 0, 0, 0);
+      __builtin_amdgcn_sched_barrier(0);
+    }
+  }
+  FF_STAMP(128, 2);
+  asm volatile("s_waitcnt lgkmcnt(0)" ::: "memory");
+  __builtin_amdgcn_s_barrier();
+  FF_STAMP(128, 3);
+  dma_mlp(0, 0);
+  if (p.HT > 1) dma_mlp(1, 1);
+#pragma unroll
+  for (int n = 0; n < 6; ++n) {
+    load_res(n);
+    const int c4 = n * 32 + q4;
+    f32x4 sc = {0.f, 0.f, 0.f, 0.f};
+    if (c4 < p.K) sc = *reinterpret_cast<const f32x4*>(p.a_rs2 + (long long)b * p.a_rs2_ld + c4);
+#pragma unroll
+    for (int i = 0; i < 4; ++i) {
+      f32x4 r0 = rx[i];
+      r0 += rc[i] * sc;
+      *reinterpret_cast<f32x4*>(patch + (tq + 8 * i) * 36 + q4) = r0;
+    }
+#pragma unroll
+    for (int g = 0; g < 4; ++g) {
+      const f32x4 u = *reinterpret_cast<const f32x4*>(patch + l31 * 36 + 8 * g + 4 * hh);
+#pragma unroll
+      for (int e = 0; e < 4; ++e) oacc[n][4 * g + e] += u[e];
+    }
+  }
+  FF_STAMP(128, 4);
+
+  {
+    float s = 0.f;
+#pragma unroll
+    for (int n = 0; n < 6; ++n)
+#pragma unroll
+      for (int r = 0; r < 16; ++r) s += (n * 32 + (r & 3) + 8 * (r >> 2) + 4 * hh < p.K) ? oacc[n][r] : 0.f;
+    s += __shfl_xor(s, 32);
+    const float mean = s / (float)p.K;
+    float qv = 0.f;
+#pragma unroll
+    for (int n = 0; n < 6; ++n)
+#pragma unroll
+      for (int r = 0; r < 16; ++r) {
+        const float d = (n * 32 + (r & 3) + 8 * (r >> 2) + 4 * hh < p.K) ? oacc[n][r] - mean : 0.f;
+        qv += d * d;
+      }
+    qv += __shfl_xor(qv, 32);
+    const float rstd = 1.0f / sqrtf(qv / (float)p.K + p.a_eps);
+#pragma unroll
+    for (int n = 0; n < 6; ++n)
+#pragma unroll
+      for (int s2 = 0; s2 < 2; ++s2) {
+#pragma unroll
+        for (int g2 = 0; g2 < 2; ++g2) {
+          const int c0 = n * 32 + 8 * (2 * s2 + g2) + 4 * hh;
+          const f32x4 g4 = *reinterpret_cast<const f32x4*>(Gs + c0);
+          const f32x4 b4 = *reinterpret_cast<const f32x4*>(Bts + c0);
+#pragma unroll
+          for (int e = 0; e < 4; ++e)
+            xh[2 * n + s2][4 * g2 + e] = (__bf16)((oacc[n][8 * s2 + 4 * g2 + e] - mean) * rstd * g4[e] + b4[e]);
+        }
+        asm volatile("" : "+v"(xh[2 * n + s2]) :: "memory");
+      }
+  }
+  FF_STAMP(128, 5);
+  asm volatile("s_waitcnt vmcnt(0) lgkmcnt(0)" ::: "memory");
+  __builtin_amdgcn_s_barrier();
+  FF_STAMP(128, 6);
+
+#define PM_STAMP(i) FF_STAMP(128, i)
+#include "token_projmlp_bf16_mlp.inc"
+#undef PM_STAMP
+  FF_STAMP(128, 40);
+
+  int woff[5];
+#pragma unroll
+  for (int i = 0; i < 5; ++i) {
+    int s = (wid + 8 * i) * 64 + lane;
+    if (s >= W2_HEAD_SLOTS) s = W2_HEAD_SLOTS - 1;
+    const int tile = s / WF_PL, t = s - tile * WF_PL, row = t / WF_SLOTS;
+    int q = t - row * WF_SLOTS;
+    if (q > 2 * WF_KS - 1) q = 2 * WF_KS - 1;
+    woff[i] = tile * (2 * WF_TILE_ELEMS) + row * 192 + q * 8;
+  }
+  const int reln = p.rel_rows * p.rel_stride;
+  const int relpieces = (reln + 255) >> 8;
+  auto dma_head = [&](int head, int buf) {
+    const __bf16* rec = p.w + (long long)(3 * head) * (2 * WF_TILE_ELEMS);
+#pragma unroll
+    for (int i = 0; i < 5; ++i)
+      if (wid + 8 * i < W2_PIECES)
+        __builtin_amdgcn_global_load_lds((const __attribute__((address_space(1))) void*)(rec + woff[i]),
+                                         (__attribute__((address_space(3))) void*)(smem + (wid + 8 * i) * 1024), 16, 0, 0);
+    const float* src = p.rel + (long long)head * reln;
+#pragma unroll
+    for (int i = 0; i < 2; ++i)
+      if (wid + 8 * i < relpieces) {
+        int c = (wid + 8 * i) * 64 + lane;
+        if (c > (reln >> 2) - 1) c = (reln >> 2) - 1;
+        __builtin_amdgcn_global_load_lds((const __attribute__((address_space(1))) void*)(src + 4 * c),
+                                         (__attribute__((address_space(3))) void*)(smem + W2_OFF_REL + buf * W2_RELB + WF_REL_PAD * 4 + (wid + 8 * i) * 1024), 16, 0, 0);
+      }
+  };
+  dma_head(0, 0);
+  for (int i = tid; i < 3 * HL_HEADS * 32; i += 512) Bs[i] = (i % 96 == 94) ? 1.0f : p.bias[i];
+
+  const bool blk_mask = p.use_mask && (wy == p.nwy - 1 || wx == p.nwx - 1);
+  const int qi = wid * 32 + 31 - l31;
+  const int mytok = tok_of(qi);
+  constexpr bool tvalid = true, kill_pad = false;
+  constexpr unsigned vmask = 0xffffffffu;
+  int qreg_id = 0;
+  if (p.use_mask) {
+    const int qy = wy * WH + qi / WW, qx = wx * WW + qi % WW;
+    const int ry = qy < p.H - WH ? 0 : (qy < p.H - p.sh ? 1 : 2);
+    const int rx2 = qx < p.W - WW ? 0 : (qx < p.W - p.sw ? 1 : 2);
+    qreg_id = 3 * ry + rx2;
+  }
+  const float msy = (qreg_id / 3 == 2) ? -7.0625f : 7.0625f, msx = (qreg_id % 3 == 2) ? -7.0625f : 7.0625f;
+
+  {
+    float* xs = reinterpret_cast<float*>(smem + W2_OFF_K) + wid * (32 * WF_XS_ROW);
+    float v[WF_KS][8];
+    int oo[4];
+#pragma unroll
+    for (int i = 0; i < 4; ++i) oo[i] = tok_of(wid * 32 + tq + 8 * i) * p.a_ldo + q4;
+    const float* xrow = xs + (31 - l31) * WF_XS_ROW + 8 * hh;
+#pragma unroll
+    for (int pass = 0; pass < 3; ++pass) {
+#pragma unroll
+      for (int h2 = 0; h2 < 2; ++h2) {
+        const int n = 2 * pass + h2;
+#pragma unroll
+        for (int g = 0; g < 4; ++g) {
+          const int c0 = n * 32 + 8 * g + 4 * hh;
+          const bool cok = c0 < p.K;
+          const f32x4 b4 = *reinterpret_cast<const f32x4*>(p.a_b2 + (cok ? c0 : 0));
+          f32x4 v4;
+#pragma unroll
+          for (int e = 0; e < 4; ++e) v4[e] = cok ? oacc[n][4 * g + e] + b4[e] : 0.f;
+          *reinterpret_cast<f32x4*>(xs + l31 * WF_XS_ROW + 32 * h2 + 8 * g + 4 * hh) = v4;
+        }
+      }
+#pragma unroll
+      for (int h2 = 0; h2 < 2; ++h2) {
+        const int cn = (2 * pass + h2) * 32;
+        f32x4 ov[4];
+#pragma unroll
+        for (int i = 0; i < 4; ++i) ov[i] = *reinterpret_cast<const f32x4*>(xs + (tq + 8 * i) * WF_XS_ROW + 32 * h2 + q4);
+        if (cn + q4 < p.K) {
+#pragma unroll
+          for (int i = 0; i < 4; ++i) *reinterpret_cast<f32x4*>(p.a_out + (oo[i] + cn)) = ov[i];
+        }
+      }
+#pragma unroll
+      for (int s4 = 0; s4 < 4; ++s4) {
+        const f32x4 a = *reinterpret_cast<const f32x4*>(xrow + 16 * s4);
+        const f32x4 c4 = *reinterpret_cast<const f32x4*>(xrow + 16 * s4 + 4);
+#pragma unroll
+        for (int e = 0; e < 4; ++e) { v[4 * pass + s4][e] = a[e]; v[4 * pass + s4][4 + e] = c4[e]; }
+      }
+    }
+    FF_STAMP(128, 41);
+    asm volatile("s_waitcnt vmcnt(0)" ::: "memory");
+    FF_STAMP(128, 42);
+#include "win_attn_fused_v2_ln.inc"
+  }
+  FF_STAMP(128, 64 + 2);
+
+#define W2_STAMP(i) FF_STAMP(128, 64 + (i))
+#include "win_attn_fused_v2_heads.inc"
+#undef W2_STAMP
+  FF_STAMP(128, 64 + 60);
+  FF_STAMP_DRAINED(128, 64 + 61);
+}
+
+static bool g_hl_attr[64];
+
+extern "C" int ff_hab_link(const float* att, int lda, const float* x, int ldx, const float* c2, int ldc, const float* c2_scale,
+                           int scale_ld, int B, long long rows_per_image, float* x_out, int ldxo, long long M, int K, int hidden_tiles,
+                           const void* proj_tiles, const float* proj_bias_padded, const float* gamma2, const float* beta2, float eps2,
+                           const void* mlp_tiles, const float* b1_padded, const float* b2, int nterms, int io_bf16,
+                           float* att_out, int ldo, int o_off, const float* gamma1, const float* beta1, float eps1,
+                           const void* qkv_tiles, const float* qkv_bias_padded, const float* rel_padded, int rel_rows, int rel_stride,
+                           int H, int W, int wh, int ww, int shift_h, int shift_w, int use_mask, int nheads, int d,
+                           float* xn_out, int ldxn, int out_bf16, int xn_bf16, void* stream) {
+  FF_CHECK_ARG(nterms == 1, "ff_hab_link: plain bf16 only (nterms must be 1)");
+  FF_CHECK_ARG(wh == 16 && ww == 16, "ff_hab_link: the window must be 16x16 (got %dx%d)", wh, ww);
+  FF_CHECK_ARG(d == 30 && nheads == HL_HEADS, "ff_hab_link: six heads of dim 30 only (got %d x %d)", nheads, d);
+  FF_CHECK_ARG(K == HL_K, "ff_hab_link: K must be 180 (got %d)", K);
+  FF_CHECK_ARG(B > 0 && H > 0 && W > 0 && H % 16 == 0 && W % 16 == 0, "ff_hab_link: H and W must be positive multiples of 16 (got %dx%d)", H, W);
+  FF_CHECK_ARG(io_bf16 == 3 && out_bf16 == 1 && xn_bf16 == 1, "ff_hab_link: att, c2, xn_out and att_out are bf16 rows (fp32 rows are refused)");
+  FF_CHECK_ARG(c2 && c2_scale, "ff_hab_link: c2 and the gate are required");
+  FF_CHECK_ARG(att && x && x_out && proj_tiles && proj_bias_padded && gamma2 && beta2 && mlp_tiles && b1_padded && b2 && att_out && gamma1 && beta1 &&
+               qkv_tiles && qkv_bias_padded && rel_padded && xn_out, "ff_hab_link: null pointer");
+  FF_CHECK_ARG(rows_per_image == (long long)H * W && M == (long long)B * rows_per_image, "ff_hab_link: rows_per_image must be H * W and M must be B * rows_per_image");
+  FF_CHECK_ARG(hidden_tiles > 0 && hidden_tiles <= 12, "ff_hab_link: at most 12 hidden tiles (got %d)", hidden_tiles);
+  FF_CHECK_ARG(lda % 8 == 0 && lda >= 192 && ldc % 4 == 0 && ldc >= K && (((uintptr_t)att) & 15) == 0 && (((uintptr_t)c2) & 7) == 0,
+               "ff_hab_link: bf16 att rows must be 16-byte aligned and padded to 192 channels, c2 rows 8-byte aligned");
+  FF_CHECK_ARG(ldx % 4 == 0 && ldx >= K && ldxo % 4 == 0 && ldxo >= K && (((uintptr_t)x) & 15) == 0 && (((uintptr_t)x_out) & 15) == 0,
+               "ff_hab_link: x / x_out rows must be 16-byte aligned");
+  FF_CHECK_ARG(scale_ld >= K && scale_ld % 4 == 0 && (((uintptr_t)c2_scale) & 15) == 0, "ff_hab_link: gate rows must be 16-byte aligned (scale_ld >= K, scale_ld %% 4 == 0)");
+  FF_CHECK_ARG(ldxn % 8 == 0 && ldxn >= 192 && (((uintptr_t)xn_out) & 15) == 0, "ff_hab_link: bf16 xn rows must be 16-byte aligned and padded to 192 channels");
+  FF_CHECK_ARG(ldo % 2 == 0 && o_off % 2 == 0 && o_off >= 0 && (((uintptr_t)att_out) & 7) == 0 && ldo >= o_off + nheads * d, "ff_hab_link: att_out rows must be 8-byte aligned and hold every head");
+  FF_CHECK_ARG((((uintptr_t)proj_tiles) & 15) == 0 && (((uintptr_t)mlp_tiles) & 15) == 0 && (((uintptr_t)qkv_tiles) & 15) == 0 && (((uintptr_t)rel_padded) & 15) == 0 &&
+               (((uintptr_t)gamma1) & 15) == 0 && (((uintptr_t)beta1) & 15) == 0 && (((uintptr_t)b2) & 15) == 0,
+               "ff_hab_link: weights / bias table / gamma1 / beta1 / b2 must be 16-byte aligned");
+  FF_CHECK_ARG(shift_h >= 0 && shift_w >= 0 && shift_h < wh && shift_w < ww, "ff_hab_link: bad shift");
+  FF_CHECK_ARG(!use_mask || (shift_h > 0 && shift_w > 0), "ff_hab_link: mask needs a shift");
+  FF_CHECK_ARG(rel_rows == 2 * wh - 1 && rel_stride == 48, "ff_hab_link: bias table must be [heads][31][stride 48]");
+  {
+    int ldmax = lda > ldx ? lda : ldx;
+    if (ldc > ldmax) ldmax = ldc;
+    if (ldxo > ldmax) ldmax = ldxo;
+    if (ldo > ldmax) ldmax = ldo;
+    if (ldxn > ldmax) ldmax = ldxn;
+    FF_CHECK_ARG(M * (long long)ldmax < (1LL << 31), "ff_hab_link: too many tokens for 32-bit row offsets (B * H * W * ld must be < 2^31)");
+  }
+  HabLinkParams p;
+  p.a_att = (const __bf16*)att; p.a_x = x; p.a_c2 = (const __bf16*)c2; p.a_rs2 = c2_scale; p.a_out = x_out;
+  p.a_gamma = gamma2; p.a_beta = beta2; p.a_wp = (const __bf16*)proj_tiles; p.a_bp = proj_bias_padded; p.a_w = (const __bf16*)mlp_tiles;
+  p.a_b1 = b1_padded; p.a_b2 = b2; p.a_lda = lda; p.a_ldx = ldx; p.a_ldc = ldc; p.a_ldo = ldxo; p.a_rs2_ld = scale_ld; p.HT = hidden_tiles;
+  p.a_eps = eps2;
+  p.out = att_out; p.gamma = gamma1; p.beta = beta1; p.w = (const __bf16*)qkv_tiles; p.bias = qkv_bias_padded; p.rel = rel_padded; p.xn = xn_out;
+  p.ldo = ldo; p.ldxn = ldxn; p.o_off = o_off; p.H = H; p.W = W; p.sh = shift_h; p.sw = shift_w; p.use_mask = use_mask;
+  p.nwx = W / ww; p.nwy = H / wh; p.rel_rows = rel_rows; p.rel_stride = rel_stride; p.eps = eps1; p.K = K;
+  FF_STAMP_ARM(p);
+  const long long nblk = (long long)B * p.nwx * p.nwy;
+  FF_CHECK_ARG(nblk < (1LL << 31), "ff_hab_link: grid too large");
+  int dev = 0;
+  hipError_t e = hipGetDevice(&dev);
+  if (e != hipSuccess || dev < 0 || dev >= 64) { ff_set_error("ff_hab_link: cannot identify the device: %s", hipGetErrorString(e)); return FF_ERR_LAUNCH; }
+  if (!g_hl_attr[dev]) {
+    e = hipFuncSetAttribute(reinterpret_cast<const void*>(&hab_link_kernel), hipFuncAttributeMaxDynamicSharedMemorySize, HL_LDS);
+    if (e != hipSuccess) { ff_set_error("ff_hab_link: cannot raise dynamic LDS: %s", hipGetErrorString(e)); return FF_ERR_LAUNCH; }
+    g_hl_attr[dev] = true;
+  }
+  hipLaunchKernelGGL(hab_link_kernel, dim3((unsigned)nblk), dim3(512), HL_LDS, (hipStream_t)stream, p);
+  FF_LAUNCH_CHECK("ff_hab_link");
+  return FF_OK;
+}
diff --git a/image-super-resolution-2_amd/csrc/token_mlp.hip b/image-super-resolution-2_amd/csrc/token_mlp.hip
--- a/image-super-resolution-2_amd/csrc/token_mlp.hip
+++ b/image-super-resolution-2_amd/csrc/token_mlp.hip
@@ -1,18 +1,6 @@
 #include "ff_common.h"
 
-#define TM_KP 192
-#define TM_NP 192
-#define TM_KS 12
-#define W1SLOTS 25
-#define W2SLOTS 5
-#define W1ROWB (W1SLOTS * 16)
-#define W2ROWB (W2SLOTS * 16)
-#define W1PL (32 * W1SLOTS)
-#define W2PL (TM_NP * W2SLOTS)
-#define W1PIECES (2 * W1PL / 64)
-#define W2PIECES (2 * W2PL / 64)
-#define TILE_ELEMS 6144
-#define XLROWB 400
+#include "token_mlp_layout.h"
 
 struct TokenMlpParams {
   const float* x; float* out;
@@ -564,13 +552,6 @@
   FF_STAMP_DRAINED(64, 42);
 }
 
-#define PM_W1SLOT (13 * 1024)
-#define PM_W2SLOT (15 * 1024)
-#define PM_OFF_W2 (2 * PM_W1SLOT)
-#define PM_PROJB (6 * PM_W1SLOT)
-#define PM_PATCHB (32 * FF_XS_ROW * 4)
-#define PM_OFF_PATCH PM_PROJB
-#define PM_OFF_VEC (PM_OFF_PATCH + 8 * PM_PATCHB)
 
 __global__ __launch_bounds__(512) void token_projmlp_bf16_kernel(TokenProjMlpParams p) {
   extern __shared__ __attribute__((aligned(16))) unsigned char smem[];
@@ -760,57 +741,9 @@
   __builtin_amdgcn_s_barrier();
   FF_STAMP(64, 6);
 
-  for (int ht = 0; ht < p.HT; ++ht) {
-    const int slot = ht & 1;
-    f32x16 hacc;
-#pragma unroll
-    for (int r = 0; r < 16; ++r) hacc[r] = B1s[ht * 32 + (r & 3) + 8 * (r >> 2) + 4 * hh];
-    {
-      const unsigned char* ap = smem + slot * PM_W1SLOT + l31 * W1ROWB + 16 * hh;
-      bf16x8 fa[2];
-#pragma unroll
-      for (int u = 0; u < 2; ++u) fa[u] = *reinterpret_cast<const bf16x8*>(ap + 32 * u);
-#pragma unroll
-      for (int st = 0; st < TM_KS; ++st) {
-        const bf16x8 ah = fa[st & 1];
-        if (st + 2 < TM_KS) fa[st & 1] = *reinterpret_cast<const bf16x8*>(ap + 32 * (st + 2));
-        __builtin_amdgcn_sched_barrier(0);
-        hacc = __builtin_amdgcn_mfma_f32_32x32x16_bf16(ah, xh[st], hacc, 0, 0, 0);
-        __builtin_amdgcn_sched_barrier(0);
-      }
-    }
-    if (ht < 3) FF_STAMP(64, 8 + 4 * ht);
-    bf16x8 gh[2];
-#pragma unroll
-    for (int s = 0; s < 2; ++s)
-#pragma unroll
-      for (int j = 0; j < 8; j += 2) {
-        const f32x2 g = ff_gelu_sig2((f32x2){hacc[8 * s + j], hacc[8 * s + j + 1]});
-        gh[s][j] = (__bf16)g[0];
-        gh[s][j + 1] = (__bf16)g[1];
-      }
-    if (ht < 3) FF_STAMP(64, 9 + 4 * ht);
-    {
-      const unsigned char* ap = smem + PM_OFF_W2 + slot * PM_W2SLOT + l31 * W2ROWB + 16 * hh;
-      bf16x8 fa[2];
-#pragma unroll
-      for (int u = 0; u < 2; ++u) fa[u] = *reinterpret_cast<const bf16x8*>(ap + (u >> 1) * 32 * W2ROWB + 32 * (u & 1));
-#pragma unroll
-      for (int u = 0; u < 12; ++u) {
-        const int n = u >> 1, s2 = u & 1;
-        const bf16x8 ah = fa[u & 1];
-        if (u + 2 < 12) fa[u & 1] = *reinterpret_cast<const bf16x8*>(ap + ((u + 2) >> 1) * 32 * W2ROWB + 32 * ((u + 2) & 1));
-        __builtin_amdgcn_sched_barrier(0);
-        oacc[n] = __builtin_amdgcn_mfma_f32_32x32x16_bf16(ah, gh[s2], oacc[n], 0, 0, 0);
-        __builtin_amdgcn_sched_barrier(0);
-      }
-    }
-    if (ht < 3) FF_STAMP(64, 10 + 4 * ht);
-    asm volatile("s_waitcnt vmcnt(0) lgkmcnt(0)" ::: "memory");
-    __builtin_amdgcn_s_barrier();
-    if (ht < 3) FF_STAMP(64, 11 + 4 * ht);
-    if (ht + 2 < p.HT) dma_mlp(ht + 2, slot);
-  }
+#define PM_STAMP(i) FF_STAMP(64, i)
+#include "token_projmlp_bf16_mlp.inc"
+#undef PM_STAMP
   FF_STAMP(64, 40);
 
   {
diff --git a/image-super-resolution-2_amd/csrc/token_mlp_layout.h b/image-super-resolution-2_amd/csrc/token_mlp_layout.h
--- /dev/null
+++ b/image-super-resolution-2_amd/csrc/token_mlp_layout.h
@@ -0,0 +1,21 @@
+#pragma once
+#define TM_KP 192
+#define TM_NP 192
+#define TM_KS 12
+#define W1SLOTS 25
+#define W2SLOTS 5
+#define W1ROWB (W1SLOTS * 16)
+#define W2ROWB (W2SLOTS * 16)
+#define W1PL (32 * W1SLOTS)
+#define W2PL (TM_NP * W2SLOTS)
+#define W1PIECES (2 * W1PL / 64)
+#define W2PIECES (2 * W2PL / 64)
+#define TILE_ELEMS 6144
+#define XLROWB 400
+#define PM_W1SLOT (13 * 1024)
+#define PM_W2SLOT (15 * 1024)
+#define PM_OFF_W2 (2 * PM_W1SLOT)
+#define PM_PROJB (6 * PM_W1SLOT)
+#define PM_PATCHB (32 * FF_XS_ROW * 4)
+#define PM_OFF_PATCH PM_PROJB
+#define PM_OFF_VEC (PM_OFF_PATCH + 8 * PM_PATCHB)
diff --git a/image-super-resolution-2_amd/csrc/token_projmlp_bf16_mlp.inc b/image-super-resolution-2_amd/csrc/token_projmlp_bf16_mlp.inc
--- /dev/null
+++ b/image-super-resolution-2_amd/csrc/token_projmlp_bf16_mlp.inc
@@ -0,0 +1,51 @@
+  for (int ht = 0; ht < p.HT; ++ht) {
+    const int slot = ht & 1;
+    f32x16 hacc;
+#pragma unroll
+    for (int r = 0; r < 16; ++r) hacc[r] = B1s[ht * 32 + (r & 3) + 8 * (r >> 2) + 4 * hh];
+    {
+      const unsigned char* ap = smem + slot * PM_W1SLOT + l31 * W1ROWB + 16 * hh;
+      bf16x8 fa[2];
+#pragma unroll
+      for (int u = 0; u < 2; ++u) fa[u] = *reinterpret_cast<const bf16x8*>(ap + 32 * u);
+#pragma unroll
+      for (int st = 0; st < TM_KS; ++st) {
+        const bf16x8 ah = fa[st & 1];
+        if (st + 2 < TM_KS) fa[st & 1] = *reinterpret_cast<const bf16x8*>(ap + 32 * (st + 2));
+        __builtin_amdgcn_sched_barrier(0);
+        hacc = __builtin_amdgcn_mfma_f32_32x32x16_bf16(ah, xh[st], hacc, 0, 0, 0);
+        __builtin_amdgcn_sched_barrier(0);
+      }
+    }
+    if (ht < 3) PM_STAMP(8 + 4 * ht);
+    bf16x8 gh[2];
+#pragma unroll
+    for (int s = 0; s < 2; ++s)
+#pragma unroll
+      for (int j = 0; j < 8; j += 2) {
+        const f32x2 g = ff_gelu_sig2((f32x2){hacc[8 * s + j], hacc[8 * s + j + 1]});
+        gh[s][j] = (__bf16)g[0];
+        gh[s][j + 1] = (__bf16)g[1];
+      }
+    if (ht < 3) PM_STAMP(9 + 4 * ht);
+    {
+      const unsigned char* ap = smem + PM_OFF_W2 + slot * PM_W2SLOT + l31 * W2ROWB + 16 * hh;
+      bf16x8 fa[2];
+#pragma unroll
+      for (int u = 0; u < 2; ++u) fa[u] = *reinterpret_cast<const bf16x8*>(ap + (u >> 1) * 32 * W2ROWB + 32 * (u & 1));
+#pragma unroll
+      for (int u = 0; u < 12; ++u) {
+        const int n = u >> 1, s2 = u & 1;
+        const bf16x8 ah = fa[u & 1];
+        if (u + 2 < 12) fa[u & 1] = *reinterpret_cast<const bf16x8*>(ap + ((u + 2) >> 1) * 32 * W2ROWB + 32 * ((u + 2) & 1));
+        __builtin_amdgcn_sched_barrier(0);
+        oacc[n] = __builtin_amdgcn_mfma_f32_32x32x16_bf16(ah, gh[s2], oacc[n], 0, 0, 0);
+        __builtin_amdgcn_sched_barrier(0);
+      }
+    }
+    if (ht < 3) PM_STAMP(10 + 4 * ht);
+    asm volatile("s_waitcnt vmcnt(0) lgkmcnt(0)" ::: "memory");
+    __builtin_amdgcn_s_barrier();
+    if (ht < 3) PM_STAMP(11 + 4 * ht);
+    if (ht + 2 < p.HT) dma_mlp(ht + 2, slot);
+  }
diff --git a/image-super-resolution-2_amd/csrc/win_attn_fused.hip b/image-super-resolution-2_amd/csrc/win_attn_fused.hip
--- a/image-super-resolution-2_amd/csrc/win_attn_fused.hip
+++ b/image-super-resolution-2_amd/csrc/win_attn_fused.hip
@@ -15,29 +15,7 @@
   FF_STAMP_MEMBER
 };
 
-#define WF_KS 12
-#define WF_SLOTS 25
-#define WF_ROWB (WF_SLOTS * 16)
-#define WF_PL (32 * WF_SLOTS)
-#define WF_PLB (WF_PL * 16)
-#define WF_BUFB (2 * WF_PLB)
-#define WF_TILE_ELEMS (32 * 192)
-#define WF_KROWB 80
-#define WF_KWAVE (2 * 32 * WF_KROWB)
-#define WF_VROWB 528
-#define WF_VPLB (32 * WF_VROWB)
-#define WF_OFF_K (2 * WF_BUFB)
-#define WF_OFF_V (WF_OFF_K + 8 * WF_KWAVE)
-#define WF_OFF_REL (WF_OFF_V + 2 * WF_VPLB)
-#define WF_REL_MAX 2560
-#define WF_REL_PAD 4
-#define WF_OFF_BS (WF_OFF_REL + (WF_REL_MAX + WF_REL_PAD) * 4)
-#define WF_BS_MAX 576
-#define WF_OFF_TOK (WF_OFF_BS + WF_BS_MAX * 4)
-#define WF_OFF_REG (WF_OFF_TOK + 1024)
-#define WF_OFF_SAME (WF_OFF_REG + 1024)
-#define WF_LDS (WF_OFF_SAME + 9 * 8 * 4)
-#define WF_XS_ROW 68
+#include "win_attn_layout.h"
 
 template <int WW, int NTERMS>
 __global__ __launch_bounds__(512) void win_attn_fused_kernel(WinFusedParams p) {
diff --git a/image-super-resolution-2_amd/csrc/win_attn_fused_v2.inc b/image-super-resolution-2_amd/csrc/win_attn_fused_v2.inc
--- a/image-super-resolution-2_amd/csrc/win_attn_fused_v2.inc
+++ b/image-super-resolution-2_amd/csrc/win_attn_fused_v2.inc
@@ -1,21 +1,3 @@
-#define W2_TILEB (32 * WF_ROWB)
-#define W2_HEAD_SLOTS (3 * WF_PL)
-#define W2_PIECES ((W2_HEAD_SLOTS + 63) / 64)
-#define W2_WB (W2_PIECES * 1024)
-#define W2_KROWB 80
-#define W2_KWAVE (32 * W2_KROWB)
-#define W2_KBUF (8 * W2_KWAVE)
-#define W2_VROWB 528
-#define W2_VBUF (32 * W2_VROWB)
-#define W2_RELB ((WF_REL_MAX + WF_REL_PAD) * 4)
-#define W2_OFF_K W2_WB
-#define W2_OFF_V (W2_OFF_K + 2 * W2_KBUF)
-#define W2_OFF_REL (W2_OFF_V + 2 * W2_VBUF)
-#define W2_OFF_BS (W2_OFF_REL + 2 * W2_RELB)
-#define W2_OFF_TOK (W2_OFF_BS + WF_BS_MAX * 4)
-#define W2_OFF_REG (W2_OFF_TOK + 1024)
-#define W2_OFF_SAME (W2_OFF_REG + 1024)
-#define W2_LDS (W2_OFF_SAME + 9 * 8 * 4)
 
 template <int WW, bool ONES>
 __global__ __launch_bounds__(512) void win_attn_fused_v2_kernel(WinFusedParams p) {
@@ -134,244 +116,13 @@
       }
     }
     asm volatile("s_waitcnt vmcnt(0)" ::: "memory");
-    float mean = 0.f, rstd = 1.f;
-    if (p.gamma) {
-      float s = 0.f;
-#pragma unroll
-      for (int st = 0; st < WF_KS; ++st)
-#pragma unroll
-        for (int j = 0; j < 8; ++j) s += v[st][j];
-      s += __shfl_xor(s, 32);
-      mean = s / (float)p.K;
-      float qv = 0.f;
-#pragma unroll
-      for (int st = 0; st < WF_KS; ++st)
-#pragma unroll
-        for (int j = 0; j < 8; ++j) {
-          const float dd = (16 * st + 8 * hh + j < p.K) ? v[st][j] - mean : 0.f;
-          qv += dd * dd;
-        }
-      qv += __shfl_xor(qv, 32);
-      rstd = 1.0f / sqrtf(qv / (float)p.K + p.eps);
-    }
-#pragma unroll
-    for (int st = 0; st < WF_KS; ++st) {
-      const int k0 = 16 * st + 8 * hh;
-      f32x4 g0 = {1.f, 1.f, 1.f, 1.f}, g1 = g0, b0 = {0.f, 0.f, 0.f, 0.f}, b1 = b0;
-      if (p.gamma) {
-        const int ka = k0 < p.K ? k0 : 0, kb = k0 + 4 < p.K ? k0 + 4 : 0;
-        g0 = *reinterpret_cast<const f32x4*>(p.gamma + ka); b0 = *reinterpret_cast<const f32x4*>(p.beta + ka);
-        g1 = *reinterpret_cast<const f32x4*>(p.gamma + kb); b1 = *reinterpret_cast<const f32x4*>(p.beta + kb);
-      }
-#pragma unroll
-      for (int j = 0; j < 8; ++j) {
-        const float gg = j < 4 ? g0[j & 3] : g1[j & 3], bb = j < 4 ? b0[j & 3] : b1[j & 3];
-        const float f = (k0 + j < p.K) ? (p.gamma ? (v[st][j] - mean) * rstd * gg + bb : v[st][j]) : 0.f;
-        xh[st][j] = (__bf16)f;
-        v[st][j] = f;
-      }
-      if (p.xn && tvalid && p.xn_bf16) {
-        if (k0 < p.K) *reinterpret_cast<bf16x8*>(reinterpret_cast<__bf16*>(p.xn) + (long long)mytok * p.ldxn + k0) = xh[st];
-      } else if (p.xn && tvalid) {
-        float* xr = p.xn + (long long)mytok * p.ldxn + k0;
-        if (k0 < p.K) *reinterpret_cast<f32x4*>(xr) = (f32x4){v[st][0], v[st][1], v[st][2], v[st][3]};
-        if (k0 + 4 < p.K) *reinterpret_cast<f32x4*>(xr + 4) = (f32x4){v[st][4], v[st][5], v[st][6], v[st][7]};
-      }
-    }
+#include "win_attn_fused_v2_ln.inc"
   }
   FF_STAMP(64, 2);
 
-  const int rel_lane = ((qi / WW) + WH - 1) * RS + (qi % WW) + WW - 1 - (TPR - 1) * RS - (WWM - 1) + 4 * hh;
-  const float LOG2E = 1.4426950408889634f;
-
-  auto gemm_tile = [&](int j, bool swap, f32x16& acc) {
-    const unsigned char* ap = smem + j * W2_TILEB + l31 * WF_ROWB + 16 * hh;
-    bf16x8 fa[2];
-#pragma unroll
-    for (int u = 0; u < 2; ++u) fa[u] = *reinterpret_cast<const bf16x8*>(ap + 32 * u);
-#pragma unroll
-    for (int st = 0; st < WF_KS; ++st) {
-      const bf16x8 ah = fa[st & 1];
-      if (st + 2 < WF_KS) fa[st & 1] = *reinterpret_cast<const bf16x8*>(ap + 32 * (st + 2));
-      __builtin_amdgcn_sched_barrier(0);
-      if (!swap) acc = __builtin_amdgcn_mfma_f32_32x32x16_bf16(ah, xh[st], acc, 0, 0, 0);
-      else acc = __builtin_amdgcn_mfma_f32_32x32x16_bf16(xh[st], ah, acc, 0, 0, 0);
-      __builtin_amdgcn_sched_barrier(0);
-    }
-  };
-
-  for (int hi = 0; hi < p.nheads; ++hi) {
-    const int g = p.head0 + hi, buf = hi & 1;
-    unsigned char* KB = smem + W2_OFF_K + buf * W2_KBUF;
-    unsigned char* VB = smem + W2_OFF_V + buf * W2_VBUF;
-    asm volatile("s_waitcnt lgkmcnt(0)" ::: "memory");
-    __builtin_amdgcn_s_barrier();
-    FF_STAMP(64, 3 + 8 * hi);
-    bf16x8 qh[2];
-    {
-      f32x16 acc;
-      const int nb = (3 * hi) * 32 + 4 * hh;
-#pragma unroll
-      for (int r = 0; r < 16; ++r) acc[r] = Bs[nb + (r & 3) + 8 * (r >> 2)];
-      gemm_tile(0, false, acc);
-      if (ONES && blk_mask && hh) { acc[14] = msy; acc[15] = msx; }
-#pragma unroll
-      for (int s = 0; s < 2; ++s)
-#pragma unroll
-        for (int j = 0; j < 8; ++j) qh[s][j] = (__bf16)acc[8 * s + j];
-    }
-    FF_STAMP(64, 4 + 8 * hi);
-    {
-      f32x16 acc;
-      const int nb = (3 * hi + 1) * 32 + 4 * hh;
-#pragma unroll
-      for (int r = 0; r < 16; ++r) acc[r] = Bs[nb + (r & 3) + 8 * (r >> 2)];
-      gemm_tile(1, false, acc);
-      const bool zero = kill_pad && !tvalid;
-      if (zero) {
-#pragma unroll
-        for (int r = 0; r < 16; ++r) acc[r] = 0.f;
-      }
-      if (ONES && blk_mask && hh) { acc[14] = msy; acc[15] = msx; }
-      unsigned char* kmine = KB + wid * W2_KWAVE + l31 * W2_KROWB + 16 * hh;
-#pragma unroll
-      for (int s = 0; s < 2; ++s) {
-        bf16x8 h8;
-#pragma unroll
-        for (int j = 0; j < 8; ++j) h8[j] = (__bf16)acc[8 * s + j];
-        *reinterpret_cast<bf16x8*>(kmine + 32 * s) = h8;
-      }
-    }
-    FF_STAMP(64, 5 + 8 * hi);
-    {
-      f32x16 acc;
-      const float bv = Bs[(3 * hi + 2) * 32 + l31];
-#pragma unroll
-      for (int r = 0; r < 16; ++r) acc[r] = bv;
-      gemm_tile(2, true, acc);
-      if (kill_pad && !(ONES && l31 == 30)) {
-#pragma unroll
-        for (int r = 0; r < 16; ++r)
-          if (!((vmask >> ((r & 3) + 8 * (r >> 2) + 4 * hh)) & 1u)) acc[r] = 0.f;
-      }
-      unsigned char* vp = VB + l31 * W2_VROWB + 64 * wid + 16 * hh;
-#pragma unroll
-      for (int s = 0; s < 2; ++s) {
-        bf16x8 h8;
-#pragma unroll
-        for (int j = 0; j < 8; ++j) h8[j] = (__bf16)acc[8 * s + j];
-        *reinterpret_cast<bf16x8*>(vp + 32 * s) = h8;
-      }
-      if (p.vout && l31 < p.d) {
-#pragma unroll
-        for (int r = 0; r < 16; ++r) {
-          const int tk = ktok[wid * 32 + 31 - ((r & 3) + 8 * (r >> 2) + 4 * hh)];
-          if (tk >= 0) p.vout[(long long)tk * p.ldv + p.v_off + g * p.d + l31] = acc[r];
-        }
-      }
-    }
-    FF_STAMP(64, 6 + 8 * hi);
-    asm volatile("s_waitcnt lgkmcnt(0)" ::: "memory");
-    __builtin_amdgcn_s_barrier();
-    FF_STAMP(64, 7 + 8 * hi);
-    if (hi + 1 < p.nheads) dma_head(g + 1, buf ^ 1);
-
-    f32x16 o;
-#pragma unroll
-    for (int r = 0; r < 16; ++r) o[r] = 0.f;
-    float m_run = -INFINITY, l_run = 0.f;
-    unsigned rel_addr = (unsigned)(size_t)(__attribute__((address_space(3))) const void*)(smem + W2_OFF_REL + buf * W2_RELB + WF_REL_PAD * 4) + 4u * (unsigned)rel_lane;
-    const unsigned char* kp = KB + l31 * W2_KROWB + 16 * hh;
-    const unsigned char* vq = VB + l31 * W2_VROWB + 16 * hh;
-    const unsigned* samep = same + 8 * qreg_id;
-#pragma unroll 2
-    for (int t = 0; t < 8; ++t, rel_addr -= 4u * TPR * RS, kp += W2_KWAVE, vq += 64) {
-      unsigned ra = rel_addr;
-      asm volatile("" : "+v"(ra));
-      const ff_lds_cf relp = (ff_lds_cf)(size_t)ra;
-      f32x16 st;
-#pragma unroll
-      for (int r = 0; r < 16; ++r) {
-        const int c = (r & 3) + 8 * (r >> 2);
-        st[r] = relp[(c / WW) * RS + (c % WW)];
-      }
-      bf16x8 vh2[2];
-#pragma unroll
-      for (int s = 0; s < 2; ++s) vh2[s] = *reinterpret_cast<const bf16x8*>(vq + 32 * s);
-#pragma unroll
-      for (int s = 0; s < 2; ++s) {
-        const bf16x8 ah = *reinterpret_cast<const bf16x8*>(kp + 32 * s);
-        st = __builtin_amdgcn_mfma_f32_32x32x16_bf16(ah, qh[s], st, 0, 0, 0);
-      }
-      if (!ONES && blk_mask) {
-        const unsigned m = samep[t] >> (4 * hh);
-#pragma unroll
-        for (int r = 0; r < 16; ++r)
-          st[r] += ((m >> ((r & 3) + 8 * (r >> 2))) & 1u) ? 0.f : -100.0f;
-      }
-      float mx = st[0];
-#pragma unroll
-      for (int r = 1; r < 16; ++r) mx = fmaxf(mx, st[r]);
-      {
-        float lo, hi;
-        ff_halves(mx, lo, hi);
-        mx = fmaxf(lo, hi);
-      }
-      if (__builtin_amdgcn_ballot_w64(mx > m_run) != 0) {
-        const float m_new = fmaxf(m_run, mx);
-        const float corr = __builtin_amdgcn_exp2f((m_run - m_new) * LOG2E);
-#pragma unroll
-        for (int r = 0; r < 16; ++r) o[r] *= corr;
-        if (!ONES) l_run *= corr;
-        m_run = m_new;
-      }
-      const float mneg = -m_run * LOG2E;
-      float ls = 0.f;
-#pragma unroll
-      for (int s = 0; s < 2; ++s) {
-        bf16x8 ph;
-#pragma unroll
-        for (int j = 0; j < 8; ++j) {
-          const float e = __builtin_amdgcn_exp2f(__builtin_fmaf(st[8 * s + j], LOG2E, mneg));
-          if (!ONES) ls += e;
-          ph[j] = (__bf16)e;
-        }
-        o = __builtin_amdgcn_mfma_f32_32x32x16_bf16(vh2[s], ph, o, 0, 0, 0);
-      }
-      if (!ONES) l_run += ls;
-    }
-    float den;
-    if (ONES) {
-      float lo;
-      ff_halves(o[14], lo, den);
-    } else {
-      den = l_run + __shfl_xor(l_run, 32);
-    }
-    const float inv = 1.0f / den;
-    FF_STAMP(64, 8 + 8 * hi);
-    asm volatile("s_waitcnt vmcnt(0)" ::: "memory");
-    FF_STAMP(64, 9 + 8 * hi);
-
-    if (tvalid && p.out_bf16) {
-      typedef __bf16 bf16x2 __attribute__((ext_vector_type(2)));
-      __bf16* orow = reinterpret_cast<__bf16*>(p.out) + (long long)mytok * p.ldo + p.o_off + g * p.d + 4 * hh;
-#pragma unroll
-      for (int i = 0; i < 4; ++i) {
-        const int c = 8 * i + 4 * hh;
-        if (c < p.d) *reinterpret_cast<bf16x2*>(orow + 8 * i) = (bf16x2){(__bf16)(o[4 * i] * inv), (__bf16)(o[4 * i + 1] * inv)};
-        if (c + 2 < p.d) *reinterpret_cast<bf16x2*>(orow + 8 * i + 2) = (bf16x2){(__bf16)(o[4 * i + 2] * inv), (__bf16)(o[4 * i + 3] * inv)};
-      }
-    } else if (tvalid) {
-      float* orow = p.out + (long long)mytok * p.ldo + p.o_off + g * p.d + 4 * hh;
-#pragma unroll
-      for (int i = 0; i < 4; ++i) {
-        const int c = 8 * i + 4 * hh;
-        if (c < p.d) *reinterpret_cast<float2*>(orow + 8 * i) = (float2){o[4 * i] * inv, o[4 * i + 1] * inv};
-        if (c + 2 < p.d) *reinterpret_cast<float2*>(orow + 8 * i + 2) = (float2){o[4 * i + 2] * inv, o[4 * i + 3] * inv};
-      }
-    }
-    FF_STAMP(64, 10 + 8 * hi);
-  }
+#define W2_STAMP(i) FF_STAMP(64, i)
+#include "win_attn_fused_v2_heads.inc"
+#undef W2_STAMP
   FF_STAMP(64, 60);
   FF_STAMP_DRAINED(64, 61);
 }
diff --git a/image-super-resolution-2_amd/csrc/win_attn_fused_v2_heads.inc b/image-super-resolution-2_amd/csrc/win_attn_fused_v2_heads.inc
--- /dev/null
+++ b/image-super-resolution-2_amd/csrc/win_attn_fused_v2_heads.inc
@@ -0,0 +1,191 @@
+  const int rel_lane = ((qi / WW) + WH - 1) * RS + (qi % WW) + WW - 1 - (TPR - 1) * RS - (WWM - 1) + 4 * hh;
+  const float LOG2E = 1.4426950408889634f;
+
+  auto gemm_tile = [&](int j, bool swap, f32x16& acc) {
+    const unsigned char* ap = smem + j * W2_TILEB + l31 * WF_ROWB + 16 * hh;
+    bf16x8 fa[2];
+#pragma unroll
+    for (int u = 0; u < 2; ++u) fa[u] = *reinterpret_cast<const bf16x8*>(ap + 32 * u);
+#pragma unroll
+    for (int st = 0; st < WF_KS; ++st) {
+      const bf16x8 ah = fa[st & 1];
+      if (st + 2 < WF_KS) fa[st & 1] = *reinterpret_cast<const bf16x8*>(ap + 32 * (st + 2));
+      __builtin_amdgcn_sched_barrier(0);
+      if (!swap) acc = __builtin_amdgcn_mfma_f32_32x32x16_bf16(ah, xh[st], acc, 0, 0, 0);
+      else acc = __builtin_amdgcn_mfma_f32_32x32x16_bf16(xh[st], ah, acc, 0, 0, 0);
+      __builtin_amdgcn_sched_barrier(0);
+    }
+  };
+
+  for (int hi = 0; hi < p.nheads; ++hi) {
+    const int g = p.head0 + hi, buf = hi & 1;
+    unsigned char* KB = smem + W2_OFF_K + buf * W2_KBUF;
+    unsigned char* VB = smem + W2_OFF_V + buf * W2_VBUF;
+    asm volatile("s_waitcnt lgkmcnt(0)" ::: "memory");
+    __builtin_amdgcn_s_barrier();
+    W2_STAMP(3 + 8 * hi);
+    bf16x8 qh[2];
+    {
+      f32x16 acc;
+      const int nb = (3 * hi) * 32 + 4 * hh;
+#pragma unroll
+      for (int r = 0; r < 16; ++r) acc[r] = Bs[nb + (r & 3) + 8 * (r >> 2)];
+      gemm_tile(0, false, acc);
+      if (ONES && blk_mask && hh) { acc[14] = msy; acc[15] = msx; }
+#pragma unroll
+      for (int s = 0; s < 2; ++s)
+#pragma unroll
+        for (int j = 0; j < 8; ++j) qh[s][j] = (__bf16)acc[8 * s + j];
+    }
+    W2_STAMP(4 + 8 * hi);
+    {
+      f32x16 acc;
+      const int nb = (3 * hi + 1) * 32 + 4 * hh;
+#pragma unroll
+      for (int r = 0; r < 16; ++r) acc[r] = Bs[nb + (r & 3) + 8 * (r >> 2)];
+      gemm_tile(1, false, acc);
+      const bool zero = kill_pad && !tvalid;
+      if (zero) {
+#pragma unroll
+        for (int r = 0; r < 16; ++r) acc[r] = 0.f;
+      }
+      if (ONES && blk_mask && hh) { acc[14] = msy; acc[15] = msx; }
+      unsigned char* kmine = KB + wid * W2_KWAVE + l31 * W2_KROWB + 16 * hh;
+#pragma unroll
+      for (int s = 0; s < 2; ++s) {
+        bf16x8 h8;
+#pragma unroll
+        for (int j = 0; j < 8; ++j) h8[j] = (__bf16)acc[8 * s + j];
+        *reinterpret_cast<bf16x8*>(kmine + 32 * s) = h8;
+      }
+    }
+    W2_STAMP(5 + 8 * hi);
+    {
+      f32x16 acc;
+      const float bv = Bs[(3 * hi + 2) * 32 + l31];
+#pragma unroll
+      for (int r = 0; r < 16; ++r) acc[r] = bv;
+      gemm_tile(2, true, acc);
+      if (kill_pad && !(ONES && l31 == 30)) {
+#pragma unroll
+        for (int r = 0; r < 16; ++r)
+          if (!((vmask >> ((r & 3) + 8 * (r >> 2) + 4 * hh)) & 1u)) acc[r] = 0.f;
+      }
+      unsigned char* vp = VB + l31 * W2_VROWB + 64 * wid + 16 * hh;
+#pragma unroll
+      for (int s = 0; s < 2; ++s) {
+        bf16x8 h8;
+#pragma unroll
+        for (int j = 0; j < 8; ++j) h8[j] = (__bf16)acc[8 * s + j];
+        *reinterpret_cast<bf16x8*>(vp + 32 * s) = h8;
+      }
+      if (p.vout && l31 < p.d) {
+#pragma unroll
+        for (int r = 0; r < 16; ++r) {
+          const int tk = ktok[wid * 32 + 31 - ((r & 3) + 8 * (r >> 2) + 4 * hh)];
+          if (tk >= 0) p.vout[(long long)tk * p.ldv + p.v_off + g * p.d + l31] = acc[r];
+        }
+      }
+    }
+    W2_STAMP(6 + 8 * hi);
+    asm volatile("s_waitcnt lgkmcnt(0)" ::: "memory");
+    __builtin_amdgcn_s_barrier();
+    W2_STAMP(7 + 8 * hi);
+    if (hi + 1 < p.nheads) dma_head(g + 1, buf ^ 1);
+
+    f32x16 o;
+#pragma unroll
+    for (int r = 0; r < 16; ++r) o[r] = 0.f;
+    float m_run = -INFINITY, l_run = 0.f;
+    unsigned rel_addr = (unsigned)(size_t)(__attribute__((address_space(3))) const void*)(smem + W2_OFF_REL + buf * W2_RELB + WF_REL_PAD * 4) + 4u * (unsigned)rel_lane;
+    const unsigned char* kp = KB + l31 * W2_KROWB + 16 * hh;
+    const unsigned char* vq = VB + l31 * W2_VROWB + 16 * hh;
+    const unsigned* samep = same + 8 * qreg_id;
+#pragma unroll 2
+    for (int t = 0; t < 8; ++t, rel_addr -= 4u * TPR * RS, kp += W2_KWAVE, vq += 64) {
+      unsigned ra = rel_addr;
+      asm volatile("" : "+v"(ra));
+      const ff_lds_cf relp = (ff_lds_cf)(size_t)ra;
+      f32x16 st;
+#pragma unroll
+      for (int r = 0; r < 16; ++r) {
+        const int c = (r & 3) + 8 * (r >> 2);
+        st[r] = relp[(c / WW) * RS + (c % WW)];
+      }
+      bf16x8 vh2[2];
+#pragma unroll
+      for (int s = 0; s < 2; ++s) vh2[s] = *reinterpret_cast<const bf16x8*>(vq + 32 * s);
+#pragma unroll
+      for (int s = 0; s < 2; ++s) {
+        const bf16x8 ah = *reinterpret_cast<const bf16x8*>(kp + 32 * s);
+        st = __builtin_amdgcn_mfma_f32_32x32x16_bf16(ah, qh[s], st, 0, 0, 0);
+      }
+      if (!ONES && blk_mask) {
+        const unsigned m = samep[t] >> (4 * hh);
+#pragma unroll
+        for (int r = 0; r < 16; ++r)
+          st[r] += ((m >> ((r & 3) + 8 * (r >> 2))) & 1u) ? 0.f : -100.0f;
+      }
+      float mx = st[0];
+#pragma unroll
+      for (int r = 1; r < 16; ++r) mx = fmaxf(mx, st[r]);
+      {
+        float lo, hi;
+        ff_halves(mx, lo, hi);
+        mx = fmaxf(lo, hi);
+      }
+      if (__builtin_amdgcn_ballot_w64(mx > m_run) != 0) {
+        const float m_new = fmaxf(m_run, mx);
+        const float corr = __builtin_amdgcn_exp2f((m_run - m_new) * LOG2E);
+#pragma unroll
+        for (int r = 0; r < 16; ++r) o[r] *= corr;
+        if (!ONES) l_run *= corr;
+        m_run = m_new;
+      }
+      const float mneg = -m_run * LOG2E;
+      float ls = 0.f;
+#pragma unroll
+      for (int s = 0; s < 2; ++s) {
+        bf16x8 ph;
+#pragma unroll
+        for (int j = 0; j < 8; ++j) {
+          const float e = __builtin_amdgcn_exp2f(__builtin_fmaf(st[8 * s + j], LOG2E, mneg));
+          if (!ONES) ls += e;
+          ph[j] = (__bf16)e;
+        }
+        o = __builtin_amdgcn_mfma_f32_32x32x16_bf16(vh2[s], ph, o, 0, 0, 0);
+      }
+      if (!ONES) l_run += ls;
+    }
+    float den;
+    if (ONES) {
+      float lo;
+      ff_halves(o[14], lo, den);
+    } else {
+      den = l_run + __shfl_xor(l_run, 32);
+    }
+    const float inv = 1.0f / den;
+    W2_STAMP(8 + 8 * hi);
+    asm volatile("s_waitcnt vmcnt(0)" ::: "memory");
+    W2_STAMP(9 + 8 * hi);
+
+    if (tvalid && p.out_bf16) {
+      typedef __bf16 bf16x2 __attribute__((ext_vector_type(2)));
+      __bf16* orow = reinterpret_cast<__bf16*>(p.out) + (long long)mytok * p.ldo + p.o_off + g * p.d + 4 * hh;
+#pragma unroll
+      for (int i = 0; i < 4; ++i) {
+        const int c = 8 * i + 4 * hh;
+        if (c < p.d) *reinterpret_cast<bf16x2*>(orow + 8 * i) = (bf16x2){(__bf16)(o[4 * i] * inv), (__bf16)(o[4 * i + 1] * inv)};
+        if (c + 2 < p.d) *reinterpret_cast<bf16x2*>(orow + 8 * i + 2) = (bf16x2){(__bf16)(o[4 * i + 2] * inv), (__bf16)(o[4 * i + 3] * inv)};
+      }
+    } else if (tvalid) {
+      float* orow = p.out + (long long)mytok * p.ldo + p.o_off + g * p.d + 4 * hh;
+#pragma unroll
+      for (int i = 0; i < 4; ++i) {
+        const int c = 8 * i + 4 * hh;
+        if (c < p.d) *reinterpret_cast<float2*>(orow + 8 * i) = (float2){o[4 * i] * inv, o[4 * i + 1] * inv};
+        if (c + 2 < p.d) *reinterpret_cast<float2*>(orow + 8 * i + 2) = (float2){o[4 * i + 2] * inv, o[4 * i + 3] * inv};
+      }
+    }
+    W2_STAMP(10 + 8 * hi);
+  }
diff --git a/image-super-resolution-2_amd/csrc/win_attn_fused_v2_ln.inc b/image-super-resolution-2_amd/csrc/win_attn_fused_v2_ln.inc
--- /dev/null
+++ b/image-super-resolution-2_amd/csrc/win_attn_fused_v2_ln.inc
@@ -0,0 +1,44 @@
+    float mean = 0.f, rstd = 1.f;
+    if (p.gamma) {
+      float s = 0.f;
+#pragma unroll
+      for (int st = 0; st < WF_KS; ++st)
+#pragma unroll
+        for (int j = 0; j < 8; ++j) s += v[st][j];
+      s += __shfl_xor(s, 32);
+      mean = s / (float)p.K;
+      float qv = 0.f;
+#pragma unroll
+      for (int st = 0; st < WF_KS; ++st)
+#pragma unroll
+        for (int j = 0; j < 8; ++j) {
+          const float dd = (16 * st + 8 * hh + j < p.K) ? v[st][j] - mean : 0.f;
+          qv += dd * dd;
+        }
+      qv += __shfl_xor(qv, 32);
+      rstd = 1.0f / sqrtf(qv / (float)p.K + p.eps);
+    }
+#pragma unroll
+    for (int st = 0; st < WF_KS; ++st) {
+      const int k0 = 16 * st + 8 * hh;
+      f32x4 g0 = {1.f, 1.f, 1.f, 1.f}, g1 = g0, b0 = {0.f, 0.f, 0.f, 0.f}, b1 = b0;
+      if (p.gamma) {
+        const int ka = k0 < p.K ? k0 : 0, kb = k0 + 4 < p.K ? k0 + 4 : 0;
+        g0 = *reinterpret_cast<const f32x4*>(p.gamma + ka); b0 = *reinterpret_cast<const f32x4*>(p.beta + ka);
+        g1 = *reinterpret_cast<const f32x4*>(p.gamma + kb); b1 = *reinterpret_cast<const f32x4*>(p.beta + kb);
+      }
+#pragma unroll
+      for (int j = 0; j < 8; ++j) {
+        const float gg = j < 4 ? g0[j & 3] : g1[j & 3], bb = j < 4 ? b0[j & 3] : b1[j & 3];
+        const float f = (k0 + j < p.K) ? (p.gamma ? (v[st][j] - mean) * rstd * gg + bb : v[st][j]) : 0.f;
+        xh[st][j] = (__bf16)f;
+        v[st][j] = f;
+      }
+      if (p.xn && tvalid && p.xn_bf16) {
+        if (k0 < p.K) *reinterpret_cast<bf16x8*>(reinterpret_cast<__bf16*>(p.xn) + (long long)mytok * p.ldxn + k0) = xh[st];
+      } else if (p.xn && tvalid) {
+        float* xr = p.xn + (long long)mytok * p.ldxn + k0;
+        if (k0 < p.K) *reinterpret_cast<f32x4*>(xr) = (f32x4){v[st][0], v[st][1], v[st][2], v[st][3]};
+        if (k0 + 4 < p.K) *reinterpret_cast<f32x4*>(xr + 4) = (f32x4){v[st][4], v[st][5], v[st][6], v[st][7]};
+      }
+    }
diff --git a/image-super-resolution-2_amd/csrc/win_attn_layout.h b/image-super-resolution-2_amd/csrc/win_attn_layout.h
--- /dev/null
+++ b/image-super-resolution-2_amd/csrc/win_attn_layout.h
@@ -0,0 +1,42 @@
+#pragma once
+#define WF_KS 12
+#define WF_SLOTS 25
+#define WF_ROWB (WF_SLOTS * 16)
+#define WF_PL (32 * WF_SLOTS)
+#define WF_PLB (WF_PL * 16)
+#define WF_BUFB (2 * WF_PLB)
+#define WF_TILE_ELEMS (32 * 192)
+#define WF_KROWB 80
+#define WF_KWAVE (2 * 32 * WF_KROWB)
+#define WF_VROWB 528
+#define WF_VPLB (32 * WF_VROWB)
+#define WF_OFF_K (2 * WF_BUFB)
+#define WF_OFF_V (WF_OFF_K + 8 * WF_KWAVE)
+#define WF_OFF_REL (WF_OFF_V + 2 * WF_VPLB)
+#define WF_REL_MAX 2560
+#define WF_REL_PAD 4
+#define WF_OFF_BS (WF_OFF_REL + (WF_REL_MAX + WF_REL_PAD) * 4)
+#define WF_BS_MAX 576
+#define WF_OFF_TOK (WF_OFF_BS + WF_BS_MAX * 4)
+#define WF_OFF_REG (WF_OFF_TOK + 1024)
+#define WF_OFF_SAME (WF_OFF_REG + 1024)
+#define WF_LDS (WF_OFF_SAME + 9 * 8 * 4)
+#define WF_XS_ROW 68
+#define W2_TILEB (32 * WF_ROWB)
+#define W2_HEAD_SLOTS (3 * WF_PL)
+#define W2_PIECES ((W2_HEAD_SLOTS + 63) / 64)
+#define W2_WB (W2_PIECES * 1024)
+#define W2_KROWB 80
+#define W2_KWAVE (32 * W2_KROWB)
+#define W2_KBUF (8 * W2_KWAVE)
+#define W2_VROWB 528
+#define W2_VBUF (32 * W2_VROWB)
+#define W2_RELB ((WF_REL_MAX + WF_REL_PAD) * 4)
+#define W2_OFF_K W2_WB
+#define W2_OFF_V (W2_OFF_K + 2 * W2_KBUF)
+#define W2_OFF_REL (W2_OFF_V + 2 * W2_VBUF)
+#define W2_OFF_BS (W2_OFF_REL + 2 * W2_RELB)
+#define W2_OFF_TOK (W2_OFF_BS + WF_BS_MAX * 4)
+#define W2_OFF_REG (W2_OFF_TOK + 1024)
+#define W2_OFF_SAME (W2_OFF_REG + 1024)
+#define W2_LDS (W2_OFF_SAME + 9 * 8 * 4)
diff --git a/image-super-resolution-2_amd/experts.py b/image-super-resolution-2_amd/experts.py
--- a/image-super-resolution-2_amd/experts.py
+++ b/image-super-resolution-2_amd/experts.py
@@ -197,10 +197,43 @@
         x = ops.linear(att, *blk["proj"], res=x)
         return self._mlp(x, blk)
 
+    def _linked(self, x: T) -> bool:
+        B, H, W, C = x.shape
+        return (ops.gemm_mode() == "bf16" and H * W >= 1024 and (self.ws, self.heads, C) == (16, 6, 180) and H % 16 == 0 and W % 16 == 0
+                and B * H * W * 192 < 2 ** 31)
+
+    def _habs_linked(self, x: T, blks: List[dict]) -> T:
+        B, H, W, C = x.shape
+        d, win = C // self.heads, (self.ws, self.ws)
+
+        def relp(blk):
+            return _packed(blk, "relp", lambda: pack_win_rel(blk["rel"], self.ws, self.ws))
+
+        s = blks[0]["shift"]
+        att = ops.empty_rows_bf16(tuple(x.shape), x.device)
+        _, xn = ops.win_attn_fused(x, att, _wf(blks[0], self.heads, d), relp(blks[0]), gamma=blks[0]["n1"][0], beta=blks[0]["n1"][1], H=H, W=W,
+                                   Hp=H, Wp=W, win=win, shift=(s, s), use_mask=s > 0, want_xn="bf16")
+        for i, blk in enumerate(blks):
+            c1 = ops.conv2d(xn, *blk["cab0"], ksize=(3, 3), pad=(1, 1), act="gelu", out_bf16=True, per_image=True)
+            c2, c2mean = ops.conv2d(c1, *blk["cab2"], ksize=(3, 3), pad=(1, 1), want_pool="partials", out_bf16=True)
+            gate = ops.vec_mlp(c2mean, *blk["ca1"], "relu", *blk["ca2"], "sigmoid", post=self.conv_scale)
+            gate = gate if B > 1 else gate.reshape(-1)
+            if i + 1 < len(blks):
+                nxt = blks[i + 1]
+                s = nxt["shift"]
+                x, xn, att = ops.hab_link(att, x, _pm(blk), blk["n2"][0], blk["n2"][1], c2=c2, c2_scale=gate, wf=_wf(nxt, self.heads, d),
+                                          rel_padded=relp(nxt), gamma1=nxt["n1"][0], beta1=nxt["n1"][1], shift=(s, s), use_mask=s > 0)
+            else:
+                x = ops.token_projmlp(att, x, _pm(blk), blk["n2"][0], blk["n2"][1], c2=c2, c2_scale=gate)
+        return x
+
     def group(self, x: T, g: int) -> T:
-        y = x
-        for blk in self.blocks[g]:
-            y = self.hab(y, blk)
+        if self._linked(x):
+            y = self._habs_linked(x, self.blocks[g])
+        else:
+            y = x
+            for blk in self.blocks[g]:
+                y = self.hab(y, blk)
         y = self.ocab_block(y, self.ocab[g])
         return ops.conv2d(y, *self.gconv[g], ksize=(3, 3), pad=(1, 1), res=x, per_image=True)
 
diff --git a/image-super-resolution-2_amd/ops.py b/image-super-resolution-2_amd/ops.py
--- a/image-super-resolution-2_amd/ops.py
+++ b/image-super-resolution-2_amd/ops.py
@@ -698,6 +698,40 @@
     return out
 
 
+def hab_link(att: T, x: T, pk: dict, gamma2: T, beta2: T, *, c2: T, c2_scale: T, wf: dict, rel_padded: T, gamma1: T, beta1: T,
+             shift: Tuple[int, int], use_mask: bool, eps2: float = 1e-5, eps1: float = 1e-5) -> Tuple[T, T, T]:
+    if _GEMM_MODE != "bf16":
+        raise _lib.FFError("hab_link exists for the plain-bf16 contraction mode only")
+    if att.dtype != torch.bfloat16 or c2 is None or c2.dtype != torch.bfloat16 or c2_scale is None:
+        raise _lib.FFError("hab_link: att and c2 must be bf16 rows, and the gate is required")
+    ap, lda, B, H, W, K = _nhwc(att, "hab_link.att|bf16ok")
+    xp, ldx, xb, xh_, xw, xk = _nhwc(x, "hab_link.x")
+    cp, ldc, cb, ch, cw, ck = _nhwc(c2, "hab_link.c2|bf16ok")
+    if (xb, xh_, xw, xk) != (B, H, W, K) or (cb, ch, cw, ck) != (B, H, W, K) or K != pk["mlp"]["K"] or K != wf["K"]:
+        raise _lib.FFError("hab_link: shape mismatch")
+    if tuple(c2_scale.shape) not in (((K,), (1, K)) if B == 1 else ((B, K),)) or not c2_scale.is_contiguous():
+        raise _lib.FFError(f"hab_link: c2_scale must be [{K}] for one image or one row per image [{B},{K}], got {tuple(c2_scale.shape)}")
+    if tuple(rel_padded.shape[:2]) != (wf["heads"], 31) or not rel_padded.is_contiguous():
+        raise _lib.FFError("hab_link: rel_padded must be [heads][31][stride]")
+    out = empty_like_rows(x)
+    op_, ldo_, *_ = _nhwc(out, "hab_link.out")
+    xn = empty_rows_bf16(tuple(x.shape), x.device)
+    xnp, ldxn, *_ = _nhwc(xn, "hab_link.xn|bf16ok")
+    ao = empty_rows_bf16(tuple(x.shape), x.device)
+    aop, ldao, *_ = _nhwc(ao, "hab_link.att_out|bf16ok")
+    m = pk["mlp"]
+    _lib.check(_L().ff_hab_link(ap, lda, xp, ldx, cp, ldc, _ptr(c2_scale), K, B, H * W, op_, ldo_, B * H * W, K, m["ht"],
+                                pk["proj"]["w"].data_ptr(), pk["proj"]["b"].data_ptr(), gamma2.data_ptr(), beta2.data_ptr(), float(eps2),
+                                m["w"].data_ptr(), m["b1"].data_ptr(), m["b2"].data_ptr(), 1, 3,
+                                aop, ldao, 0, gamma1.data_ptr(), beta1.data_ptr(), float(eps1), wf["w"].data_ptr(), wf["b"].data_ptr(),
+                                rel_padded.data_ptr(), rel_padded.shape[1], rel_padded.shape[2], H, W, 16, 16, shift[0], shift[1],
+                                int(use_mask), wf["heads"], wf["d"], xnp, ldxn, 1, 1, _stream()))
+    rows, nwin, nh, d = B * H * W, B * (H // 16) * (W // 16), wf["heads"], wf["d"]
+    _note(2.0 * rows * K * K + 4.0 * rows * K * m["ht"] * 32 + 2.0 * nwin * 256 * K * 3 * nh * d + 4.0 * nwin * nh * 256 * 256 * d,
+          4.0 * rows * K * 3.0 + 4.0 * rows * (K * 0.5 + nh * d * 0.5))
+    return out, xn, ao
+
+
 def token_linear(x: T, pk: dict, *, gamma: Optional[T] = None, beta: Optional[T] = None, eps: float = 1e-5, act=None,
                  res: Optional[T] = None, res2: Optional[T] = None, res2_scale: Optional[T] = None, want_xn: bool = False,
                  stats_range: Optional[Tuple[int, int]] = None, stats_eps: float = 1e-5):
@@ -1522,7 +1556,7 @@
     return out
 
 
-for _n in ("conv2d", "sgfn_tail", "ocab_attn", "ocab_attn_rows16", "token_linear_rows16", "linear", "win_attn_fused", "token_projmlp", "token_linear_gated", "token_mlp", "token_linear", "pixel_mlp", "dwconv3_gate_pool", "naf_front", "naf_ffn", "naf_tail", "window_attn", "layernorm", "pool_mean", "vec_mlp", "dwconv2d", "dwconv3x3_ln", "mix2", "fma3", "affine",
+for _n in ("conv2d", "sgfn_tail", "ocab_attn", "ocab_attn_rows16", "token_linear_rows16", "linear", "win_attn_fused", "token_projmlp", "hab_link", "token_linear_gated", "token_mlp", "token_linear", "pixel_mlp", "dwconv3_gate_pool", "naf_front", "naf_ffn", "naf_tail", "window_attn", "layernorm", "pool_mean", "vec_mlp", "dwconv2d", "dwconv3x3_ln", "mix2", "fma3", "affine",
            "nchw_to_nhwc", "nhwc_to_nchw", "resize", "avgpool2", "dct8_bands", "dwt_pass", "fft_bands", "chan_attn_weights", "chan_qkv_attn",
            "band_mha_core", "band_weight", "freq_guidance", "dynamic_gates", "fuse_blend", "tile_accum", "tile_normalize"):
     globals()[_n] = _instrument(globals()[_n])
diff --git a/include/ff_kernels.h b/include/ff_kernels.h
--- a/include/ff_kernels.h
+++ b/include/ff_kernels.h
@@ -68,6 +68,15 @@
                       int rel_stride, int B, int H, int W, int Hp, int Wp, int wh, int ww, int shift_h, int shift_w,
                       int use_mask, int head0, int nheads, int d, int K, int zero_pad_tokens, float* xn_out, int ldxn,
                       float* v_out, int ldv, int v_off, int nterms, int out_bf16, int xn_bf16, void* stream);
+
+int ff_hab_link(const float* att, int lda, const float* x, int ldx, const float* c2, int ldc, const float* c2_scale,
+                int scale_ld, int B, long long rows_per_image, float* x_out, int ldxo, long long M, int K, int hidden_tiles,
+                const void* proj_tiles, const float* proj_bias_padded, const float* gamma2, const float* beta2, float eps2,
+                const void* mlp_tiles, const float* b1_padded, const float* b2, int nterms, int io_bf16,
+                float* att_out, int ldo, int o_off, const float* gamma1, const float* beta1, float eps1,
+                const void* qkv_tiles, const float* qkv_bias_padded, const float* rel_padded, int rel_rows, int rel_stride,
+                int H, int W, int wh, int ww, int shift_h, int shift_w, int use_mask, int nheads, int d,
+                float* xn_out, int ldxn, int out_bf16, int xn_bf16, void* stream);
 
 int ff_token_mlp(const float* x, int ldx, float* out, int ldo, long long M, int K, int hidden_tiles, int N,
                  const float* gamma, const float* beta, float eps, const void* w_tiles, const float* b1_padded,
```

Measured after the change: 27.45 output MPix/s, median of 6. 1.02x the previous value.
